# Lukeasargen/Show-Attend-and-Tell-Pytorch-Lightning

Hardware: AMD Instinct MI355X
Metric: captions/sec (train step) at B=128, 256px, seq_len=22 (higher is better)
Workload: dtype bf16; 1 GPU; C2: resnet50 encoder_size=7 encoder_dim=512 vocab=6400 T=22, 128 images/GPU x R=5 captions, trainable encoder, Adam, full lengths, decoder_tf=always; global_batch_images=128, parallelism=dp1, grad_bucket_dtype=fp32

## Files before the change

include/sat_hip.h:

```cpp
#ifndef SAT_HIP_H
#define SAT_HIP_H
#include <stddef.h>
#include <stdint.h>

#ifdef __cplusplus
extern "C" {
#endif

#define SAT_HIP_ABI_VERSION 23

int sat_abi_version(void);
int sat_debug_trace_launches(int32_t on);
int sat_debug_option(const char* name, int32_t value);
const char* sat_last_error(void);

typedef struct sat_profile_entry {
    char name[96];
    int64_t launches;
    double total_ms;
    double flops;
    double bytes;
} sat_profile_entry;
int sat_profile_start(void);
int sat_profile_start_only(const char* name);
int sat_profile_pause(int32_t paused);
int sat_profile_stop(sat_profile_entry* out, int32_t max_entries, int32_t* n_out);

typedef struct sat_gemm_desc {
    const float* A; int64_t lda; const int32_t* a_rows;
    const float* B; int64_t ldb;
    float* C; int64_t ldc;       const int32_t* c_rows;
    int32_t M, N, K;
    int32_t amode, bmode;
    int32_t accumulate;
    int32_t epi;
    const float* bias; const float* e0; int64_t lde0; int32_t c0, c1;
    float* slab; int64_t slab_elems;
} sat_gemm_desc;
int sat_gemm_f32(const sat_gemm_desc* d, void* stream);
typedef struct sat_gemm_types { int32_t a_bf16, b_bf16, c_bf16, bf16_mfma; } sat_gemm_types;
int sat_gemm_ex(const sat_gemm_desc* d, const sat_gemm_types* t, void* stream);

typedef struct sat_decoder_dims {
    int32_t B;
    int32_t R;
    int32_t T;
    int32_t L;
    int32_t D;
    int32_t A;
    int32_t m;
    int32_t n;
    int32_t V;
    int32_t P;
    int32_t deep_output;
    int32_t padding_idx;
    int32_t precision;
    int32_t layers;
    float embed_max_norm;
    float dropout;
    float embedding_dropout;
    uint64_t dropout_seed;
} sat_decoder_dims;

#define SAT_MAX_LSTM_LAYERS 4
typedef struct sat_decoder_params {
    float* embedding;
    float* init_f_w; float* init_f_b;
    float* init_i_w; float* init_i_b;
    float* w_ih; float* w_hh;
    float* b_ih; float* b_hh;
    float* att_enc;
    float* att_dec;
    float* att_f;
    float* beta_w; float* beta_b;
    float* out_hidden;
    float* out_context;
    float* out_w; float* out_b;
    float* up_w_ih[SAT_MAX_LSTM_LAYERS - 1]; float* up_w_hh[SAT_MAX_LSTM_LAYERS - 1];
    float* up_b_ih[SAT_MAX_LSTM_LAYERS - 1]; float* up_b_hh[SAT_MAX_LSTM_LAYERS - 1];
} sat_decoder_params;

typedef struct sat_decoder_batch {
    const float* ann;
    const int32_t* caps;
    const int32_t* lengths;
    const int32_t* prow;
    const int32_t* src_row;
    const int32_t* step_offsets_host;
    const int32_t* teacher_host;
} sat_decoder_batch;

size_t sat_decoder_workspace_bytes(const sat_decoder_dims* d);

int sat_decoder_train_fwd(const sat_decoder_dims* d, const sat_decoder_params* w, const sat_decoder_batch* b,
                          float* logits_packed, float* alphas, void* workspace, size_t workspace_bytes, void* stream);

int sat_decoder_train_bwd(const sat_decoder_dims* d, const sat_decoder_params* w, const sat_decoder_batch* b,
                          const float* dlogits_packed, const float* alphas , const float* dalphas,
                          const sat_decoder_params* g, float* dann, void* workspace, size_t workspace_bytes, void* stream);

int sat_decoder_train_bwd_fork(const sat_decoder_dims* d, const sat_decoder_params* w, const sat_decoder_batch* b,
                               const float* dlogits_packed, const float* alphas, const float* dalphas, const sat_decoder_params* g,
                               float* dann, void* workspace, size_t workspace_bytes, void* side_stream, void* event, void* stream);

int sat_ce_label_smooth_fwd(const float* logits, const int32_t* targets, int32_t P, int32_t V, float smoothing,
                            float* lse_rows, float* loss_rows, int32_t* correct_rows, float* out, void* stream);
int sat_ce_label_smooth_bwd(const float* logits, const int32_t* targets, const float* lse_rows, int32_t P, int32_t V,
                            float smoothing, const float* gscale, float* dlogits, void* stream);
int sat_doubly_stochastic_fwd(const float* alphas, int32_t N, int32_t T1, int32_t L, float gamma,
                              float* asum, float* part, float* out, void* stream);
int sat_doubly_stochastic_bwd(const float* asum, const float* gscale, int32_t N, int32_t T1, int32_t L, float gamma,
                              float* dalphas, void* stream);

int sat_policy_nll_fwd(const float* logits, const int32_t* targets, const float* row_weight, int32_t P, int32_t V, float inv_temperature,
                       const int32_t* masked_ids, int32_t n_first_rows, float scale, float* lse_rows, float* logq_rows, float* out, void* stream);
int sat_policy_nll_bwd(const float* logits, const int32_t* targets, const float* row_weight, const float* lse_rows, int32_t P, int32_t V,
                       float inv_temperature, const int32_t* masked_ids, int32_t n_first_rows, float scale, const float* gscale, float* dlogits,
                       void* stream);
#define SAT_SCST_BASELINE_GREEDY 0
#define SAT_SCST_BASELINE_MEAN 1
#define SAT_SCST_MAX_SAMPLES 256
int sat_scst_prepare(const int32_t* cap_tokens, const int32_t* cap_len, const double* scores, const double* scores_greedy , int32_t B,
                     int32_t K, int32_t S, double w_cider, double w_rouge, int32_t baseline_mode, const int32_t* special_ids_host, float* reward,
                     float* baseline , float* advantage, int32_t* caps, int32_t* lengths, float* step_weight, int32_t* count,
                     void* stream);

int sat_distill_fwd(const float* logits, const float* const* teachers, const float* weights, int32_t members, int32_t combine, const int32_t* targets,
                    int32_t P, int32_t V, float inv_tau, float alpha, float smoothing, float* lse_rows, float* teacher_lse_rows, float* cnorm_rows,
                    float* loss_rows, int32_t* correct_rows, float* out, float* dlogits , void* stream);
int sat_distill_bwd(const float* logits, const float* const* teachers, const float* weights, int32_t members, int32_t combine, const int32_t* targets,
                    int32_t P, int32_t V, float inv_tau, float alpha, float smoothing, const float* lse_rows, const float* teacher_lse_rows,
                    const float* cnorm_rows, const float* gscale, int32_t dlogits_from_fwd, float* dlogits, void* stream);

#define SAT_TEMPERATURE_MAX 8
size_t sat_temperature_workspace_bytes(int32_t P, int32_t V);
int sat_temperature_nll(const float* logits, const int32_t* targets, int32_t P, int32_t V, const float* temperatures,
                        int32_t n_temperatures, float* loss_out, float* grad_out, void* workspace, void* stream);
int sat_temperature_fit(const float* logits, const int32_t* targets, int32_t P, int32_t V, float init, float lr, float momentum,
                        int32_t nesterov, int32_t iters, float* t_trace, float* loss_trace, void* workspace, void* stream);

size_t sat_decoder_infer_workspace_bytes(const sat_decoder_dims* d, int32_t max_beams);
int sat_decoder_infer_begin(const sat_decoder_dims* d, const sat_decoder_params* w, const float* ann , int32_t beams,
                            int32_t max_beams, float* h , float* c, void* workspace, size_t workspace_bytes, void* stream);
int sat_decoder_infer_step(const sat_decoder_dims* d, const sat_decoder_params* w, const float* ann, const int32_t* tokens, int32_t beams,
                           int32_t max_beams, float* h, float* c, float* logits , float* alpha ,
// ... 489 lines not shown
```

show-attend-and-tell-pytorch-lightning_amd/_lib.py:

```python
import ctypes as C
import weakref
import os

import torch

_HERE = os.path.dirname(os.path.abspath(__file__))
LIB_PATH = os.path.join(_HERE, "libsat_hip.so")
_lib = None

f32p = C.POINTER(C.c_float)
i32p = C.POINTER(C.c_int32)


class GemmDesc(C.Structure):
    _fields_ = [("A", C.c_void_p), ("lda", C.c_int64), ("a_rows", C.c_void_p),
                ("B", C.c_void_p), ("ldb", C.c_int64),
                ("C", C.c_void_p), ("ldc", C.c_int64), ("c_rows", C.c_void_p),
                ("M", C.c_int32), ("N", C.c_int32), ("K", C.c_int32),
                ("amode", C.c_int32), ("bmode", C.c_int32), ("accumulate", C.c_int32), ("epi", C.c_int32),
                ("bias", C.c_void_p), ("e0", C.c_void_p), ("lde0", C.c_int64), ("c0", C.c_int32), ("c1", C.c_int32),
                ("slab", C.c_void_p), ("slab_elems", C.c_int64)]


class DecoderDims(C.Structure):
# ... 92 lines not shown


class BeamSearchOut(C.Structure):
    _fields_ = [(k, C.c_void_p) for k in SEARCH_OUTPUTS]


class ImageDesc(C.Structure):
    _fields_ = [("offset", C.c_int64)] + [(k, C.c_int32) for k in ("height", "width", "crop_top", "crop_left", "crop_h", "crop_w", "resized_h",
                                                                  "resized_w", "out_top", "out_left", "flip", "reserved")]


class ImageJitter(C.Structure):
    _fields_ = [("order", C.c_int32 * 4), ("brightness", C.c_float), ("contrast", C.c_float), ("saturation", C.c_float), ("hue_shift", C.c_int32)]


class ImageWarp(C.Structure):
    _fields_ = [("kind", C.c_int32), ("reserved", C.c_int32), ("coeffs", C.c_double * 8)]


class JpegDesc(C.Structure):
    _fields_ = [(k, C.c_int64) for k in ("data_offset", "data_bytes", "segments_offset", "out_offset", "block_offset")] + \
               [(k, C.c_int32) for k in ("height", "width", "components", "h_samp", "v_samp", "restart_interval", "n_segments", "segment_base")] + \
               [(k, C.c_int32 * 3) for k in ("quant", "dc_table", "ac_table")] + [("reserved", C.c_int32)]


class JpegDecodeOpts(C.Structure):
    _fields_ = [("subseq_bytes", C.c_int32), ("reserved", C.c_int32), ("parallel_min_bytes", C.c_int64), ("info", C.c_void_p)]


class JpegScan(C.Structure):
    _fields_ = [(k, C.c_int64) for k in ("data_offset", "data_bytes", "segments_offset")] + \
               [("picture", C.c_int32), ("level", C.c_int32), ("n_components", C.c_int32), ("component", C.c_int32 * 3)] + \
               [(k, C.c_int32) for k in ("ss", "se", "ah", "al")] + [("dc_table", C.c_int32 * 3), ("ac_table", C.c_int32)] + \
               [(k, C.c_int32) for k in ("restart_interval", "n_segments", "segment_base", "reserved")]


class JpegQTable(C.Structure):
    _fields_ = [("q", C.c_uint16 * 64)]


class JpegHTable(C.Structure):
    _fields_ = [("lookup", C.c_uint16 * 512), ("maxcode", C.c_int32 * 18), ("valoffset", C.c_int32 * 18), ("huffval", C.c_uint8 * 256)]


class DecoderBatch(C.Structure):
    _fields_ = [("ann", C.c_void_p), ("caps", C.c_void_p), ("lengths", C.c_void_p), ("prow", C.c_void_p), ("src_row", C.c_void_p),
                ("step_offsets_host", C.c_void_p), ("teacher_host", C.c_void_p)]


SYMBOLS = {
    "sat_abi_version": (C.c_int, []),
    "sat_debug_trace_launches": (C.c_int, [C.c_int32]),
    "sat_debug_option": (C.c_int, [C.c_char_p, C.c_int32]),
    "sat_last_error": (C.c_char_p, []),
    "sat_gemm_f32": (C.c_int, [C.POINTER(GemmDesc), C.c_void_p]),
    "sat_decoder_workspace_bytes": (C.c_size_t, [C.POINTER(DecoderDims)]),
    "sat_decoder_train_fwd": (C.c_int, [C.POINTER(DecoderDims), C.POINTER(DecoderParams), C.POINTER(DecoderBatch),
                                        C.c_void_p, C.c_void_p, C.c_void_p, C.c_size_t, C.c_void_p]),
    "sat_decoder_train_bwd": (C.c_int, [C.POINTER(DecoderDims), C.POINTER(DecoderParams), C.POINTER(DecoderBatch),
                                        C.c_void_p, C.c_void_p, C.c_void_p, C.POINTER(DecoderParams), C.c_void_p,
                                        C.c_void_p, C.c_size_t, C.c_void_p]),
    "sat_decoder_train_bwd_fork": (C.c_int, [C.POINTER(DecoderDims), C.POINTER(DecoderParams), C.POINTER(DecoderBatch),
                                             C.c_void_p, C.c_void_p, C.c_void_p, C.POINTER(DecoderParams), C.c_void_p,
                                             C.c_void_p, C.c_size_t, C.c_void_p, C.c_void_p, C.c_void_p]),
    "sat_ce_label_smooth_fwd": (C.c_int, [C.c_void_p, C.c_void_p, C.c_int32, C.c_int32, C.c_float, C.c_void_p, C.c_void_p,
                                          C.c_void_p, C.c_void_p, C.c_void_p]),
    "sat_ce_label_smooth_bwd": (C.c_int, [C.c_void_p, C.c_void_p, C.c_void_p, C.c_int32, C.c_int32, C.c_float, C.c_void_p,
                                          C.c_void_p, C.c_void_p]),
    "sat_doubly_stochastic_fwd": (C.c_int, [C.c_void_p, C.c_int32, C.c_int32, C.c_int32, C.c_float, C.c_void_p, C.c_void_p,
                                            C.c_void_p, C.c_void_p]),
    "sat_doubly_stochastic_bwd": (C.c_int, [C.c_void_p, C.c_void_p, C.c_int32, C.c_int32, C.c_int32, C.c_float, C.c_void_p, C.c_void_p]),
    "sat_attention_precompute": (C.c_int, [C.c_void_p, C.c_void_p, C.c_void_p, C.c_int32, C.c_int32, C.c_int32, C.c_int32, C.c_void_p]),
    "sat_attention_step_fwd": (C.c_int, [C.c_void_p, C.c_void_p, C.c_void_p, C.c_int32, C.c_void_p, C.c_void_p, C.c_int32,
                                         C.c_void_p, C.c_int32, C.c_void_p, C.c_void_p, C.c_int32, C.c_int32, C.c_int32,
                                         C.c_int32, C.c_int32, C.c_void_p]),
}


class GemmTypes(C.Structure):
    _fields_ = [(k, C.c_int32) for k in ("a_bf16", "b_bf16", "c_bf16", "bf16_mfma")]


class ConvGeom(C.Structure):
    _fields_ = [(k, C.c_int32) for k in ("N", "H", "W", "C", "K", "R", "S", "stride", "pad", "stride_w")]


class BlockDesc(C.Structure):
    _fields_ = ([(k, C.c_int32) for k in ("kind", "stride", "cin", "mid", "cout", "has_ds", "N", "H", "W", "fwd_res_bn", "dgrad_join", "bn_bwd_epilogue")] +
                [(k, C.c_void_p) for k in ("w1", "w2", "w3", "wd")] +
                [("gamma", C.c_void_p * 4), ("beta", C.c_void_p * 4), ("running_mean", C.c_void_p * 4), ("running_var", C.c_void_p * 4),
                 ("eps", C.c_float * 4), ("momentum", C.c_float * 4)] +
                [(k, C.c_void_p) for k in ("dw1", "dw2", "dw3", "dwd")] + [("dgamma", C.c_void_p * 4), ("dbeta", C.c_void_p * 4)])


_vp, _i32, _i64, _f = C.c_void_p, C.c_int32, C.c_int64, C.c_float
SYMBOLS.update({
    "sat_encoder_blocks_arena_bytes": (C.c_size_t, [C.POINTER(BlockDesc), _i32]),
    "sat_encoder_blocks_fwd": (C.c_int, [C.POINTER(BlockDesc), _i32, _vp, _vp, C.c_size_t, _vp, C.POINTER(C.c_void_p), _vp]),
    "sat_encoder_blocks_bwd": (C.c_int, [C.POINTER(BlockDesc), _i32, _i32, _i32, _vp, _vp, C.c_size_t, _vp, _vp, _i32, _vp, _vp, _i64, _vp, _i64, _vp, _vp,
                                         C.POINTER(C.c_void_p), C.POINTER(C.c_void_p), C.POINTER(C.c_int32), _vp]),
    "sat_conv2d_fwd": (C.c_int, [_vp, _vp, _vp, _vp, C.POINTER(ConvGeom), _vp]),
    "sat_conv2d_dgrad": (C.c_int, [_vp, _vp, _vp, C.POINTER(ConvGeom), _i32, _vp]),
    "sat_conv2d_wgrad": (C.c_int, [_vp, _vp, _vp, C.POINTER(ConvGeom), _vp, _i64, _vp]),
    "sat_conv2d_wgrad_slab_bytes": (C.c_size_t, [C.POINTER(ConvGeom)]),
    "sat_conv2d_fwd_bf16": (C.c_int, [_vp, _vp, _vp, _vp, C.POINTER(ConvGeom), _vp]),
    "sat_conv2d_dgrad_bf16": (C.c_int, [_vp, _vp, _vp, C.POINTER(ConvGeom), _i32, _vp]),
    "sat_conv2d_wgrad_bf16": (C.c_int, [_vp, _vp, _vp, C.POINTER(ConvGeom), _vp, _i64, _vp]),
    "sat_gemm_ex": (C.c_int, [C.POINTER(GemmDesc), C.POINTER(GemmTypes), _vp]),
    "sat_image_normalize_nhwc4": (C.c_int, [_vp, _vp, _i32, _i32, _i32, C.POINTER(C.c_float), C.POINTER(C.c_float), _vp]),
# ... 286 lines not shown
```

show-attend-and-tell-pytorch-lightning_amd/csrc/api.hip:

```cpp
#include <stdarg.h>

#include "../../include/sat_hip.h"
#include "decoder.h"
#include "gemm.h"
#include "gemm_bf16_common.h"
#include "temperature.h"
#include "caption_score.h"

namespace sat {
static thread_local char g_err[512] = {0};
int& dev_switch(int which) {
    static int v[SW_COUNT] = {0 , getenv("SAT_NO_WGRAD3X3") ? !atoi(getenv("SAT_NO_WGRAD3X3")) : 1,
                              getenv("SAT_REDUCE_Z16") ? atoi(getenv("SAT_REDUCE_Z16")) : 1, getenv("SAT_WIDE_TILES") ? atoi(getenv("SAT_WIDE_TILES")) : 0,
                              getenv("SAT_BN_ONEPASS") ? atoi(getenv("SAT_BN_ONEPASS")) : 1,
                              getenv("SAT_BN_VPT") ? atoi(getenv("SAT_BN_VPT")) : 2,
                              getenv("SAT_ACC_PREFETCH") ? atoi(getenv("SAT_ACC_PREFETCH")) : 0};
    return v[which];
}
int& trace_launches() { static int on = getenv("SAT_TRACE_LAUNCH") ? 1 : 0; return on; }
char* last_error_buf() { return g_err; }
int fail(int code, const char* fmt, ...) {
    va_list ap; va_start(ap, fmt); vsnprintf(g_err, sizeof g_err, fmt, ap); va_end(ap);
    return code;
}
}

using namespace sat;

extern "C" {

int sat_abi_version(void) { return SAT_HIP_ABI_VERSION; }
int sat_debug_trace_launches(int32_t on) { sat::trace_launches() = on ? 1 : 0; return SAT_OK; }
int sat_debug_option(const char* name, int32_t value) {
    if (!name) return fail(SAT_EINVAL, "debug_option: null name");
    if (!strcmp(name, "wgrad3x3")) { dev_switch(SW_WGRAD3X3) = value; return SAT_OK; }
    if (!strcmp(name, "reduce_z16")) { dev_switch(SW_REDUCE_Z16) = value; return SAT_OK; }
    if (!strcmp(name, "acc_prefetch")) { dev_switch(SW_ACC_PREFETCH) = value; return SAT_OK; }
    if (!strcmp(name, "bn_vpt")) { dev_switch(SW_BN_VPT) = value; return SAT_OK; }
    if (!strcmp(name, "bn_onepass")) { dev_switch(SW_BN_ONEPASS) = value; return SAT_OK; }
    if (!strcmp(name, "wide_tiles")) { dev_switch(SW_WIDE_TILES) = value; return SAT_OK; }
    if (!strcmp(name, "glds_tile")) { glds_force_tile() = value; return SAT_OK; }
    if (!strcmp(name, "glds_stages8")) { glds_stages8() = value; return SAT_OK; }
    if (!strcmp(name, "glds_tall_k")) { glds_tall_k() = value; return SAT_OK; }
    if (!strcmp(name, "glds_tall_conv")) { glds_tall_conv() = value; return SAT_OK; }
    if (!strcmp(name, "tile_override")) { gemm_tile_override() = value; return SAT_OK; }
    return fail(SAT_EINVAL, "debug_option: unknown option %s", name);
}
const char* sat_last_error(void) { return last_error_buf(); }

static int gemm_from_desc(const sat_gemm_desc* d, const sat_gemm_types* t, void* stream);
int sat_gemm_f32(const sat_gemm_desc* d, void* stream) { return gemm_from_desc(d, nullptr, stream); }
int sat_gemm_ex(const sat_gemm_desc* d, const sat_gemm_types* t, void* stream) {
    if (!t) return fail(SAT_EINVAL, "sat_gemm_ex: null type descriptor");
    return gemm_from_desc(d, t, stream);
}
static int gemm_from_desc(const sat_gemm_desc* d, const sat_gemm_types* t, void* stream) {
    if (!d) return fail(SAT_EINVAL, "sat_gemm_f32: null descriptor");
    if (d->amode != A_ROW && d->amode != A_KMAJOR) return fail(SAT_EINVAL, "sat_gemm_f32: amode %d (dense modes only)", d->amode);
    if (d->bmode != B_ROW && d->bmode != B_KMAJOR) return fail(SAT_EINVAL, "sat_gemm_f32: bmode %d (dense modes only)", d->bmode);
    GemmArgs g;
    g.A = d->A; g.lda = d->lda; g.a_rows = d->a_rows; g.B = d->B; g.ldb = d->ldb; g.C = d->C; g.ldc = d->ldc; g.c_rows = d->c_rows;
    g.M = d->M; g.N = d->N; g.K = d->K; g.amode = d->amode; g.bmode = d->bmode; g.accumulate = d->accumulate; g.epi = d->epi;
    g.bias = d->bias; g.e0 = d->e0; g.lde0 = d->lde0; g.c0 = d->c0; g.c1 = d->c1; g.slab = d->slab; g.slab_elems = d->slab_elems;
    if (t) { g.a_bf16 = t->a_bf16; g.b_bf16 = t->b_bf16; g.c_bf16 = t->c_bf16; g.bf16_mfma = t->bf16_mfma; }
    return launch_gemm(g, (hipStream_t)stream);
}

size_t sat_decoder_workspace_bytes(const sat_decoder_dims* d) {
    if (check_dims(d) != SAT_OK) return 0;
    return decoder_workspace_bytes(*d);
}

static int check_params(const sat_decoder_dims* d, const sat_decoder_params* w, const char* what) {
    if (!w) return fail(SAT_EINVAL, "%s: null parameter struct", what);
    if (!w->embedding || !w->init_f_w || !w->init_f_b || !w->init_i_w || !w->init_i_b || !w->w_ih || !w->w_hh || !w->b_ih || !w->b_hh ||
        !w->att_enc || !w->att_dec || !w->att_f || !w->beta_w || !w->beta_b || !w->out_hidden || !w->out_w)
        return fail(SAT_EINVAL, "%s: null tensor in parameter struct", what);
    if (d->deep_output && !w->out_context) return fail(SAT_EINVAL, "%s: deep output needs output.context.weight", what);
    for (int l = 1; l < d->layers; ++l)
        if (!w->up_w_ih[l - 1] || !w->up_w_hh[l - 1] || !w->up_b_ih[l - 1] || !w->up_b_hh[l - 1])
            return fail(SAT_EINVAL, "%s: null tensor for LSTM layer %d", what, l);
    return SAT_OK;
}
static int check_batch(const sat_decoder_batch* b) {
    if (!b || !b->ann || !b->caps || !b->lengths || !b->prow || !b->src_row || !b->step_offsets_host || !b->teacher_host)
        return fail(SAT_EINVAL, "decoder: null field in batch struct");
    return SAT_OK;
}

int sat_decoder_train_fwd(const sat_decoder_dims* d, const sat_decoder_params* w, const sat_decoder_batch* b, float* logits_packed,
                          float* alphas, void* workspace, size_t workspace_bytes, void* stream) {
    SAT_TRY(check_dims(d)); SAT_TRY(check_params(d, w, "decoder_train_fwd")); SAT_TRY(check_batch(b));
    if (!alphas || !workspace || (d->P > 0 && !logits_packed)) return fail(SAT_EINVAL, "decoder_train_fwd: null output/workspace");
    return decoder_fwd(*d, *w, *b, logits_packed, alphas, (char*)workspace, workspace_bytes, (hipStream_t)stream);
}

int sat_decoder_train_bwd(const sat_decoder_dims* d, const sat_decoder_params* w, const sat_decoder_batch* b, const float* dlogits_packed,
                          const float* alphas, const float* dalphas, const sat_decoder_params* g, float* dann, void* workspace,
                          size_t workspace_bytes, void* stream) {
    SAT_TRY(check_dims(d)); SAT_TRY(check_params(d, w, "decoder_train_bwd")); SAT_TRY(check_params(d, g, "decoder_train_bwd(grads)")); SAT_TRY(check_batch(b));
    if (!alphas || !dann || !workspace || (d->P > 0 && !dlogits_packed)) return fail(SAT_EINVAL, "decoder_train_bwd: null input/output/workspace");
    return decoder_bwd(*d, *w, *b, dlogits_packed, alphas, dalphas, *g, dann, (char*)workspace, workspace_bytes, (hipStream_t)stream);
}

int sat_decoder_train_bwd_fork(const sat_decoder_dims* d, const sat_decoder_params* w, const sat_decoder_batch* b, const float* dlogits_packed,
                               const float* alphas, const float* dalphas, const sat_decoder_params* g, float* dann, void* workspace,
                               size_t workspace_bytes, void* side_stream, void* event, void* stream) {
    SAT_TRY(check_dims(d)); SAT_TRY(check_params(d, w, "decoder_train_bwd_fork")); SAT_TRY(check_params(d, g, "decoder_train_bwd_fork(grads)")); SAT_TRY(check_batch(b));
    if (!alphas || !dann || !workspace || (d->P > 0 && !dlogits_packed)) return fail(SAT_EINVAL, "decoder_train_bwd_fork: null input/output/workspace");
    if ((side_stream != nullptr) != (event != nullptr)) return fail(SAT_EINVAL, "decoder_train_bwd_fork: side stream and event go together (got %s only)", side_stream ? "a stream" : "an event");
    if (side_stream && side_stream == stream) return fail(SAT_EINVAL, "decoder_train_bwd_fork: the side stream is the caller's stream");
    if (workspace_bytes < decoder_workspace_bytes(*d))
        return fail(SAT_EINVAL, "decoder_train_bwd_fork: workspace %zu < %zu bytes", workspace_bytes, decoder_workspace_bytes(*d));
    return decoder_bwd(*d, *w, *b, dlogits_packed, alphas, dalphas, *g, dann, (char*)workspace, workspace_bytes, (hipStream_t)stream, (hipStream_t)side_stream,
                       (hipEvent_t)event);
}

int sat_ce_label_smooth_fwd(const float* logits, const int32_t* targets, int32_t P, int32_t V, float smoothing, float* lse_rows,
                            float* loss_rows, int32_t* correct_rows, float* out, void* stream) {
    if (!logits || !targets || !lse_rows || !loss_rows || !correct_rows || !out) return fail(SAT_EINVAL, "ce_label_smooth_fwd: null pointer");
    return ce_fwd(logits, targets, P, V, smoothing, lse_rows, loss_rows, correct_rows, out, (hipStream_t)stream);
}
int sat_ce_label_smooth_bwd(const float* logits, const int32_t* targets, const float* lse_rows, int32_t P, int32_t V, float smoothing,
// ... 496 lines not shown
```

show-attend-and-tell-pytorch-lightning_amd/csrc/decoder.h:

```cpp
#pragma once
#include "../../include/sat_hip.h"
#include "common.h"

namespace sat {
struct Ws;
int check_dims(const sat_decoder_dims* d);
size_t decoder_workspace_bytes(const sat_decoder_dims& d);
int decoder_fwd(const sat_decoder_dims& d, const sat_decoder_params& p, const sat_decoder_batch& b, float* logits, float* alphas,
                char* ws, size_t ws_bytes, hipStream_t st);
int decoder_bwd(const sat_decoder_dims& d, const sat_decoder_params& p, const sat_decoder_batch& b, const float* dlogits,
                const float* alphas, const float* dalphas, const sat_decoder_params& g, float* dann, char* ws, size_t ws_bytes, hipStream_t st,
                hipStream_t side = nullptr, hipEvent_t fork_event = nullptr);
enum { ATT_OP_FWD = 0, ATT_OP_BWD = 1, ATT_OP_CONTEXT_BWD = 2 };
enum { ATT_FORM_SPLIT = 0, ATT_FORM_SINGLE = 1 };
enum : unsigned { ATT_HAS_SCRATCH = 1, ATT_ANN_ALIGNED = 2, ATT_ROWS_ALIGNED = 4, ATT_HAS_BF16 = 8 };
struct AttPlan {
    int form = 0, rn = 0, passes = 0;
    int vw = 0, dchunk = 0;
    int nq = 0, lq = 0;
    size_t lds0 = 0, lds1 = 0;
};
int attention_plan(int op, int R, int L, int D, int A, int hc_ld, int T1, unsigned flags, AttPlan& plan, const char* who);
int launch_attention_fwd(hipStream_t st, const float* ann, const float* U, const float* hc, int hc_ld, const float* wf,
                         const int* lengths, int step, float* alphas, int T1, float* Z, float* XZ, int B, int R, int L, int D, int A, float* sc, void* xzb,
                         const void* annb);
size_t decoder_infer_workspace_bytes(const sat_decoder_dims& d, int Kmax);
int decoder_infer_begin(const sat_decoder_dims& d, const sat_decoder_params& p, const float* ann, int K, int Kmax, float* h, float* c,
                        char* ws, size_t ws_bytes, hipStream_t st);
int decoder_infer_step(const sat_decoder_dims& d, const sat_decoder_params& p, const float* ann, const int* tokens, int K, int Kmax,
                       float* h, float* c, float* logits, float* alpha, const float* h_noise, char* ws, size_t ws_bytes, hipStream_t st);
size_t decoder_beam_workspace_bytes(const sat_decoder_dims& d, int K, int topg, int hist_stride, int groups);
int beam_groups_check(const sat_beam_groups* g, const char* what);
bool beam_history_on(const sat_beam_history* h);
int beam_history_check(const sat_beam_history* h, int max_gen_length, const char* what);
int beam_search_workspace_bytes(const sat_beam_search_desc& s, size_t& total);
int beam_search(const sat_beam_search_desc& s, const sat_beam_search_out& o, char* ws, size_t ws_bytes, hipStream_t st);
int beam_required_check(const sat_beam_required* r, int K, int max_gen_length, const char* what);
int beam_ensemble_check_weights(const float* weight, int members, int combine, const char* what);
int beam_ensemble_check(const sat_beam_ensemble* e, const char* what);
size_t decoder_beam_ensemble_workspace_bytes(const sat_beam_ensemble& e, int K, int hist_stride);
int beam_ensemble_scores(const float* const* logits, const float* weight, int members, int combine, int rows, int V, float temperature, float* combined,
                         hipStream_t st);
int launch_attention_bwd(hipStream_t st, const float* ann, const float* U, const float* hc, int hc_ld, const float* wf, const int* lengths, int step,
                         const float* alphas, const float* dalphas, int T1, const float* Z, const float* dZ, const float* dXZ, float* DZ, float* dhc,
                         int dhc_ld, float* dU, float* dwf_part, float* da, int B, int R, int L, int D, int A, void* dhcb, const void* annb);
int attention_context_bwd(const float* alphas, const float* DZ, const int* lengths, float* dann, int accumulate, int B, int R, int T1, int L, int D, hipStream_t st);
int lstm_cell_fwd(const float* x, int in, const float* h_prev, const float* c_prev, const float* w_ih, const float* w_hh, const float* b_ih, const float* b_hh,
                  float* gates, float* h_new, float* c_new, float* bias_scratch, int N, int n, hipStream_t st);
int lstm_cell_bwd(const float* x, int in, const float* h_prev, const float* c_prev, const float* c_new, const float* gates, const float* dh_new, const float* dc_new,
                  const float* w_ih, const float* w_hh, float* dx, float* dh_prev, float* dc_prev, float* dw_ih, float* dw_hh, float* db_ih, float* db_hh,
                  float* dgates, float* scratch, int N, int n, hipStream_t st);
int deep_output_fwd(const float* prev_embed, const float* hidden, const float* context, const float* w_hidden, const float* w_context, const float* w_out,
                    const float* b_out, float dropout, unsigned long long seed, float* u, float* udrop, float* logits, int N, int m, int n, int D, int V, hipStream_t st);
int deep_output_bwd(const float* dlogits, const float* hidden, const float* context, const float* u, const float* udrop, const float* w_hidden, const float* w_context,
                    const float* w_out, float dropout, unsigned long long seed, float* d_prev_embed, float* d_hidden, float* d_context, float* dw_hidden,
                    float* dw_context, float* dw_out, float* db_out, float* scratch, int N, int m, int n, int D, int V, hipStream_t st);
int init_lstm_fwd(const float* ann, const float* w_f, const float* b_f, const float* w_i, const float* b_i, float dropout, unsigned long long seed, float* mean,
                  float* f, float* init, int N, int L, int D, int m, int n2, hipStream_t st);
int init_lstm_bwd(const float* dinit, const float* mean, const float* f, const float* w_f, const float* w_i, float dropout, unsigned long long seed, float* dw_f,
                  float* db_f, float* dw_i, float* db_i, float* dann, float* df, float* dmean, float* scratch, int N, int L, int D, int m, int n2, hipStream_t st);
int embedding_fwd(float* table, const int* tokens, float* out, int rows, int V, int m, float max_norm, int* flags, hipStream_t st);
int embedding_bwd(const float* dY, const int* tokens, float* dtable, int rows, int V, int m, int padding_idx, int* scratch, hipStream_t st);
int sigmoid_bwd(const float* dy, const float* y, float* dpre, long n, hipStream_t st);
int beam_scores(const float* logits, int K, int V, float temperature, const int* masked, int n_masked, const float* parent, float* scores, hipStream_t st);
int beam_history_scores(const float* logits, int rows, int V, float temperature, const int* masked, int n_masked, const float* parent, const int* hist,
                        const int* hist_len, int hist_stride, const sat_beam_history& rules, int step, int end_id, float* scores, hipStream_t st);
int beam_group_select(const float* scores, const int* klive, int B, int K, int G, int V, int first_step, float lambda, float* work, float* values, int* indices,
                      hipStream_t st);
int beam_required_select(const float* scores, const int* klive, int B, int K, int V, const int* hist, int hist_stride, int hist_len, int first_step,
                         const sat_beam_required& req, int end_id, float* work, float* values, int* indices, hipStream_t st);
int topk(const float* x, float* work, long n, int k, float* values, int* indices, hipStream_t st);
int nucleus_keys(const float* scores, int rows, int V, float topp, float step, unsigned long long seed, unsigned long long stream, const float* gumbel,
                 float* keys, int* nucleus_size, hipStream_t st);
int colsum_public(const float* x, long ld, long rows, int cols, float* out, float* scratch, hipStream_t st);
int ce_fwd(const float* logits, const int* targets, int P, int V, float smoothing, float* lse_rows, float* loss_rows, int* correct_rows, float* out, hipStream_t st);
int ce_bwd(const float* logits, const int* targets, const float* lse_rows, int P, int V, float smoothing, const float* gscale, float* dlogits, hipStream_t st);
int ds_fwd(const float* alphas, int N, int T1, int L, float gamma, float* asum, float* part, float* out, hipStream_t st);
int ds_bwd(const float* asum, const float* gscale, int N, int T1, int L, float gamma, float* dalphas, hipStream_t st);
}
```

show-attend-and-tell-pytorch-lightning_amd/csrc/decoder.hip:

```cpp
#include "../../include/sat_hip.h"
#include <stdlib.h>
#include <map>
#include <mutex>
#include <utility>
#include "decoder_step.h"
#include "profile.h"
#include "decoder_kernels.h"

namespace sat {

struct Ws {
    size_t total = 0;
    float *U, *mean, *f, *init_img, *H_all, *C_all, *HC, *Z, *XZ, *Y, *GY, *Uact, *Wcat, *bcat;
    float *Udrop, *mean_rows, *f_rows, *init_rows, *df_rows;
    float *GU, *DGU, *bup;
    __bf16 *Wb_out, *Ub;
    __bf16 *annb;
    __bf16 *Hb, *XZb, *Wcat_b, *Wz_b, *DHCb;
    int* Tok; int* flags;
    int *emb_count, *emb_offset, *emb_cursor, *emb_list;
    float *SC, *DA;
    float *dA, *dHout, *dZout, *DZ, *DHC, *dXZ, *dHc, *dCc, *dU, *dwf_part, *dY, *colpart, *dinit_img, *df, *dmean, *slab;
    float *dmean_rows;
    float *colpart2, *slab2;
    char *zero_begin, *zero_end;
    long slab_elems;
};

Ws layout(const sat_decoder_dims& d, char* base) {
    Ws w; size_t off = 0;
    const long N = (long)d.B * d.R, T1 = d.T - 1, HCW = d.A + d.D + 4L * d.n;
    auto take = [&](size_t elems, size_t esz = 4) { size_t o = off; off += (elems * esz + 255) & ~(size_t)255; return base ? base + o : (char*)nullptr; };
    w.U = (float*)take((size_t)d.B * d.L * d.A);
    w.mean = (float*)take((size_t)d.B * d.D);
    w.f = (float*)take((size_t)d.B * d.m);
    const int NL = d.layers;
    w.init_img = (float*)take((size_t)d.B * 2 * d.n * NL);
    w.H_all = (float*)take((size_t)NL * (T1 + 1) * N * d.n);
    w.C_all = (float*)take((size_t)NL * (T1 + 1) * N * d.n);
    w.GU = w.DGU = w.bup = nullptr;
    if (NL > 1) {
        w.GU = (float*)take((size_t)(NL - 1) * T1 * N * 4 * d.n); w.DGU = (float*)take((size_t)(NL - 1) * T1 * N * 4 * d.n);
        w.bup = (float*)take((size_t)(NL - 1) * 4 * d.n);
    }
    w.HC = (float*)take((size_t)T1 * N * HCW);
    w.Z = (float*)take((size_t)T1 * N * d.D);
    w.XZ = (float*)take((size_t)T1 * N * d.D);
    w.Y = (float*)take((size_t)T1 * N * d.m);
    w.GY = (float*)take((size_t)T1 * N * 4 * d.n);
    w.Uact = (float*)take((size_t)(d.P > 0 ? d.P : 1) * d.m);
    w.Wcat = (float*)take((size_t)HCW * d.n);
    w.bcat = (float*)take((size_t)HCW);
    w.Tok = (int*)take((size_t)T1 * N);
    w.Udrop = w.mean_rows = w.f_rows = w.init_rows = w.df_rows = w.dmean_rows = nullptr;
// ... 18 lines not shown
    w.emb_list = (int*)take((size_t)T1 * N);
    w.SC = (float*)take((size_t)N * d.L); w.DA = (float*)take((size_t)N * d.L);
    w.dA = (float*)take((size_t)(d.P > 0 ? d.P : 1) * d.m);
    w.DZ = (float*)take((size_t)T1 * N * d.D);
    w.DHC = (float*)take((size_t)T1 * N * HCW);
    w.dXZ = (float*)take((size_t)N * d.D);
    w.dHout = (float*)take((size_t)T1 * N * d.n); w.zero_begin = (char*)w.dHout;
    w.dZout = (float*)take((size_t)T1 * N * d.D);
    w.dHc = (float*)take((size_t)NL * N * d.n);
    w.dCc = (float*)take((size_t)NL * N * d.n);
    w.dU = (float*)take((size_t)d.B * d.L * d.A);
    w.dwf_part = (float*)take((size_t)d.B * d.A);
    w.zero_end = base ? base + off : (char*)nullptr;
    w.dY = (float*)take((size_t)T1 * N * d.m);
    long maxrows = d.P > T1 * N ? d.P : T1 * N; if (maxrows < d.B * (long)d.L) maxrows = d.B * (long)d.L;
    long maxcols = d.V > HCW ? d.V : HCW;
    w.colpart = (float*)take((size_t)cdiv(maxrows, 256) * maxcols);
    w.dinit_img = (float*)take((size_t)d.B * 2 * d.n * NL);
    w.df = (float*)take((size_t)d.B * d.m);
    w.dmean = (float*)take((size_t)d.B * d.D);
    w.slab_elems = 8L << 20;
    w.slab = (float*)take((size_t)w.slab_elems);
    w.colpart2 = (float*)take((size_t)cdiv(maxrows, 256) * maxcols);
    w.slab2 = (float*)take((size_t)w.slab_elems);
    w.total = off;
    return w;
}

int check_dims(const sat_decoder_dims* d) {
    SAT_REQUIRE(d, "decoder: null dims");
    SAT_REQUIRE(d->B > 0 && d->R > 0 && d->T >= 2 && d->L > 0 && d->D > 0 && d->A > 0 && d->m > 0 && d->n > 0 && d->V > 0,
                "decoder: non-positive dimension (B=%d R=%d T=%d L=%d D=%d A=%d m=%d n=%d V=%d)", d->B, d->R, d->T, d->L, d->D, d->A, d->m, d->n, d->V);
    SAT_REQUIRE(d->P >= 0 && (long)d->P <= (long)d->B * d->R * (d->T - 1), "decoder: packed token count %d out of range", d->P);
    SAT_REQUIRE(d->layers >= 1 && d->layers <= SAT_MAX_LSTM_LAYERS, "decoder: layers=%d outside 1..%d", d->layers, SAT_MAX_LSTM_LAYERS);
    SAT_REQUIRE(d->dropout >= 0.f && d->dropout < 1.f && d->embedding_dropout >= 0.f && d->embedding_dropout < 1.f, "decoder: dropout must lie in [0,1)");
    return SAT_OK;
}

thread_local int t_bf16_mfma = 0;

static int cast_bf16(hipStream_t st, const float* src, __bf16* dst, long n) {
    hipLaunchKernelGGL(cast_bf16_kernel, dim3(cdiv(n / 4, 256)), dim3(256), 0, st, src, dst, n / 4);
    return launch_ok("cast_bf16");
}
static int gemm_bb_nt(hipStream_t st, const __bf16* A, long lda, const __bf16* B, long ldb, float* C, long ldc, int M, int N, int K, int epi, const float* bias,
                      int acc = 0, int c0 = 0, int c1 = 0) {
    GemmArgs g;
    g.A = A; g.lda = lda; g.B = B; g.ldb = ldb; g.C = C; g.ldc = ldc; g.M = M; g.N = N; g.K = K;
    g.amode = A_ROW; g.bmode = B_ROW; g.epi = epi; g.bias = bias; g.a_bf16 = g.b_bf16 = 1; g.c_bf16 = 0; g.bf16_mfma = 1;
    g.accumulate = acc; g.c0 = c0; g.c1 = c1;
    return launch_gemm(g, st);
}

static int gemm_bb_nn(hipStream_t st, const __bf16* A, long lda, const __bf16* B, long ldb, float* C, long ldc, int M, int N, int K, int acc, float* slab, long slab_elems) {
    GemmArgs g;
    g.A = A; g.lda = lda; g.B = B; g.ldb = ldb; g.C = C; g.ldc = ldc; g.M = M; g.N = N; g.K = K;
    g.amode = A_ROW; g.bmode = B_KMAJOR; g.a_bf16 = g.b_bf16 = 1; g.c_bf16 = 0; g.bf16_mfma = 1; g.accumulate = acc; g.slab = slab; g.slab_elems = slab_elems;
    return launch_gemm(g, st);
}

static int colsum(hipStream_t st, const Ws& w, const float* x, long ld, int rows, int cols, float* out, int accumulate = 0, float scale = 1.f) {
    if (cols <= 0) return SAT_OK;
    if (rows <= 0) { if (!accumulate) SAT_TRY(dev_fill_bytes(st, out, 0, (size_t)cols * 4)); return SAT_OK; }
    int nparts = cdiv(rows, 256);
    if (cols % 4 == 0 && ld % 4 == 0 && (reinterpret_cast<uintptr_t>(x) & 15) == 0)
        hipLaunchKernelGGL(colsum_part4_kernel, dim3(cdiv(cols / 4, 128), nparts), dim3(128), 0, st, x, ld, rows, cols / 4, 256, w.colpart);
    else
        hipLaunchKernelGGL(colsum_part_kernel, dim3(cdiv(cols, 256), nparts), dim3(256), 0, st, x, ld, rows, cols, 256, w.colpart);
    SAT_TRY(launch_ok("colsum_part"));
    hipLaunchKernelGGL(colsum_finish_kernel, dim3(cdiv(cols, 256)), dim3(256), 0, st, w.colpart, nparts, cols, out, accumulate, scale);
    return launch_ok("colsum_finish");
}

int pack_step_weights(const sat_decoder_dims& d, const sat_decoder_params& p, float* Wcat, __bf16* Wcat_b, float* bcat, float* bup, hipStream_t st) {
    const int n = d.n, HCW = d.A + d.D + 4 * n;
    hipLaunchKernelGGL(pack_wcat_kernel, dim3(cdiv((long)HCW * n + HCW, 256)), dim3(256), 0, st, p.att_dec, p.beta_w, p.w_hh, p.beta_b, p.b_ih, p.b_hh, Wcat, Wcat_b,
                       bcat, d.A, d.D, n);
    SAT_TRY(launch_ok("pack Wcat"));
    for (int l = 1; l < d.layers; ++l) {
        hipLaunchKernelGGL(add_kernel, dim3(cdiv(4 * n, 256)), dim3(256), 0, st, bup + (long)(l - 1) * 4 * n, p.up_b_ih[l - 1], p.up_b_hh[l - 1], (long)4 * n);
        SAT_TRY(launch_ok("bias add (stacked layer)"));
    }
    return SAT_OK;
}
int image_begin(const sat_decoder_dims& d, const sat_decoder_params& p, const float* ann, int images, float* U, float* mean, float* f, float* init_img,
                hipStream_t st) {
    const int n2 = 2 * d.n * d.layers;
    SAT_TRY(gemm(st, A_ROW, B_ROW, ann, d.D, p.att_enc, d.D, U, d.A, images * d.L, d.A, d.D));
    hipLaunchKernelGGL(ann_mean_kernel, dim3(images), dim3(256), 0, st, ann, mean, d.L, d.D);
    SAT_TRY(launch_ok("ann_mean"));
    if (!f) return SAT_OK;
    SAT_TRY(gemm(st, A_ROW, B_ROW, mean, d.D, p.init_f_w, d.D, f, d.m, images, d.m, d.D, 0, EPI_BIAS, p.init_f_b));
    return gemm(st, A_ROW, B_ROW, f, d.m, p.init_i_w, d.m, init_img, n2, images, n2, d.m, 0, EPI_BIAS, p.init_i_b);
}
int lstm_cell_pointwise(float* gates, int g_ld, const float* c_prev, const float* h_prev, float* c_new, float* h_new, const int* live, int rows, int n,
                        hipStream_t st) {
    hipLaunchKernelGGL(lstm_cell_fwd_kernel, dim3(cdiv((long)rows * n, 256)), dim3(256), 0, st, gates, g_ld, (const float*)nullptr, c_prev, h_prev, c_new, h_new, live,
                       0, rows, n, (__bf16*)nullptr);
    return launch_ok("lstm_cell_fwd");
}

static int live_steps(const sat_decoder_dims& d, const sat_decoder_batch& b) {
    const int T1 = d.T - 1; int ts = 0;
    for (int t = 0; t < T1; ++t) if (b.step_offsets_host[t + 1] > b.step_offsets_host[t]) ts = t + 1;
    return ts;
}

static size_t att_fwd_lds(int L, int A, int vw) { return (size_t)(ATT_RMAX * L + ATT_RMAX * A + A + ATT_RMAX * ATT_THREADS * vw) * 4; }
static size_t att_bwd_lds(int L, int A, int D) { return (size_t)(2 * ATT_RMAX * L + ATT_RMAX * A + A + ATT_RMAX * D + ATTB_WAVES * ATT_RMAX * A + ATTB_WAVES * A) * 4; }

// ... 82 lines not shown

int launch_attention_fwd(hipStream_t st, const float* ann, const float* U, const float* hc, int hc_ld, const float* wf,
                                const int* lengths, int step, float* alphas, int T1, float* Z, float* XZ, int B, int R, int L, int D, int A, float* sc, void* xzb_v,
                                const void* annb_v) {
    __bf16* xzb = reinterpret_cast<__bf16*>(xzb_v);
    const __bf16* annb = reinterpret_cast<const __bf16*>(annb_v);
    static const int no_split = getenv("SAT_ATT_FUSED") ? atoi(getenv("SAT_ATT_FUSED")) : 0;
    const unsigned flags = (sc && !no_split ? ATT_HAS_SCRATCH : 0u) | (al16(ann) && (!annb || al8(annb)) ? ATT_ANN_ALIGNED : 0u) |
                           (al16(hc) && al16(Z) && al16(XZ) ? ATT_ROWS_ALIGNED : 0u) | (xzb || annb ? ATT_HAS_BF16 : 0u);
    AttPlan pl;
    SAT_TRY(attention_plan(ATT_OP_FWD, R, L, D, A, hc_ld, T1, flags, pl, "attention_fwd"));
    if (pl.form == ATT_FORM_SPLIT) {
        switch (pl.rn) {
            case 1: return annb ? attention_fwd_split<1, __bf16>(st, annb, U, hc, hc_ld, wf, lengths, step, alphas, T1, Z, XZ, B, R, L, D, A, sc, xzb, pl)
                                : attention_fwd_split<1, float>(st, ann, U, hc, hc_ld, wf, lengths, step, alphas, T1, Z, XZ, B, R, L, D, A, sc, xzb, pl);
            case 2: return annb ? attention_fwd_split<2, __bf16>(st, annb, U, hc, hc_ld, wf, lengths, step, alphas, T1, Z, XZ, B, R, L, D, A, sc, xzb, pl)
                                : attention_fwd_split<2, float>(st, ann, U, hc, hc_ld, wf, lengths, step, alphas, T1, Z, XZ, B, R, L, D, A, sc, xzb, pl);
            case 3: return annb ? attention_fwd_split<3, __bf16>(st, annb, U, hc, hc_ld, wf, lengths, step, alphas, T1, Z, XZ, B, R, L, D, A, sc, xzb, pl)
                                : attention_fwd_split<3, float>(st, ann, U, hc, hc_ld, wf, lengths, step, alphas, T1, Z, XZ, B, R, L, D, A, sc, xzb, pl);
            case 4: return annb ? attention_fwd_split<4, __bf16>(st, annb, U, hc, hc_ld, wf, lengths, step, alphas, T1, Z, XZ, B, R, L, D, A, sc, xzb, pl)
                                : attention_fwd_split<4, float>(st, ann, U, hc, hc_ld, wf, lengths, step, alphas, T1, Z, XZ, B, R, L, D, A, sc, xzb, pl);
            case 5: return annb ? attention_fwd_split<5, __bf16>(st, annb, U, hc, hc_ld, wf, lengths, step, alphas, T1, Z, XZ, B, R, L, D, A, sc, xzb, pl)
                                : attention_fwd_split<5, float>(st, ann, U, hc, hc_ld, wf, lengths, step, alphas, T1, Z, XZ, B, R, L, D, A, sc, xzb, pl);
            case 6: return annb ? attention_fwd_split<6, __bf16>(st, annb, U, hc, hc_ld, wf, lengths, step, alphas, T1, Z, XZ, B, R, L, D, A, sc, xzb, pl)
                                : attention_fwd_split<6, float>(st, ann, U, hc, hc_ld, wf, lengths, step, alphas, T1, Z, XZ, B, R, L, D, A, sc, xzb, pl);
            case 7: return annb ? attention_fwd_split<7, __bf16>(st, annb, U, hc, hc_ld, wf, lengths, step, alphas, T1, Z, XZ, B, R, L, D, A, sc, xzb, pl)
                                : attention_fwd_split<7, float>(st, ann, U, hc, hc_ld, wf, lengths, step, alphas, T1, Z, XZ, B, R, L, D, A, sc, xzb, pl);
            default: return annb ? attention_fwd_split<8, __bf16>(st, annb, U, hc, hc_ld, wf, lengths, step, alphas, T1, Z, XZ, B, R, L, D, A, sc, xzb, pl)
                                 : attention_fwd_split<8, float>(st, ann, U, hc, hc_ld, wf, lengths, step, alphas, T1, Z, XZ, B, R, L, D, A, sc, xzb, pl);
        }
    }
    const bool vec = pl.vw == 4;
    const int dchunk = pl.dchunk;
    const size_t lds = pl.lds0;
    dim3 grid(B, cdiv(D, dchunk));
    const int RN = pl.rn;
#define SAT_ATTF(VWV, RNV)                                                                                                                  \
    case RNV:                                                                                                                               \
        SAT_TRY(ensure_dynamic_lds(reinterpret_cast<const void*>(attention_fwd_kernel<VWV, RNV>), lds)); \
        hipLaunchKernelGGL((attention_fwd_kernel<VWV, RNV>), grid, dim3(ATTF_THREADS), lds, st, ann, U, hc, hc_ld, wf, lengths, step, alphas, T1, Z, XZ, R, L, D, A, dchunk); \
        break;
    if (vec) {
        switch (RN) { SAT_ATTF(4, 1) SAT_ATTF(4, 2) SAT_ATTF(4, 3) SAT_ATTF(4, 4) SAT_ATTF(4, 5) SAT_ATTF(4, 6) SAT_ATTF(4, 7) SAT_ATTF(4, 8) default: break; }
    } else {
        switch (RN) { SAT_ATTF(1, 1) SAT_ATTF(1, 2) SAT_ATTF(1, 3) SAT_ATTF(1, 4) SAT_ATTF(1, 5) SAT_ATTF(1, 6) SAT_ATTF(1, 7) SAT_ATTF(1, 8) default: break; }
    }
#undef SAT_ATTF
    return launch_ok("attention_fwd");
}

template <int RN, typename TA>
static int attention_bwd_split_t(hipStream_t st, const TA* ann, const float* U, const float* hc, int hc_ld, const float* wf, const int* lengths, int step,
                                 const float* alphas, const float* dalphas, int T1, const float* Zs, const float* dZ_out, const float* dXZ, float* DZ, float* dhc,
                                 int dhc_ld, float* dU, float* dwf_part, float* da, int B, int R, int L, int D, int A, __bf16* dhcb, const AttPlan& pl) {
    const size_t lds_a = pl.lds0, lds_t = pl.lds1;
    SAT_TRY(ensure_dynamic_lds(reinterpret_cast<const void*>(attention_bwd_dalpha_kernel<RN, TA>), lds_a));
    SAT_TRY(ensure_dynamic_lds(reinterpret_cast<const void*>(attention_bwd_tanh_kernel<RN>), lds_t));
    const double N = (double)B * R;
    {
        ProfScope prof("attention_bwd_dalpha", 2.0 * N * L * D, (double)sizeof(TA) * B * L * D + 4.0 * N * (5.0 * D + 2.0 * L), st);
        hipLaunchKernelGGL((attention_bwd_dalpha_kernel<RN, TA>), dim3(B, cdiv(L, 16)), dim3(1024), lds_a, st, ann, hc, hc_ld, lengths, step, dalphas, T1, Zs, dZ_out, dXZ, DZ, dhc,
                           dhc_ld, da, R, L, D, A, dhcb);
        SAT_TRY(launch_ok("attention_bwd_dalpha"));
    }
    ProfScope prof("attention_bwd_tanh", 4.0 * N * L * A, 4.0 * (3.0 * B * L * A + N * (2.0 * A + 2.0 * L)), st);
    hipLaunchKernelGGL(attention_bwd_tanh_kernel<RN>, dim3(B, cdiv(A, ATTB_KCH)), dim3(1024), lds_t, st, U, hc, hc_ld, wf, lengths, step, alphas, T1, da, dhc, dhc_ld, dU,
                       dwf_part, R, L, A, dhcb);
    return launch_ok("attention_bwd_tanh");
}
int launch_attention_bwd(hipStream_t st, const float* ann, const float* U, const float* hc, int hc_ld, const float* wf, const int* lengths, int step,
                         const float* alphas, const float* dalphas, int T1, const float* Zs, const float* dZ_out, const float* dXZ, float* DZ, float* dhc,
                         int dhc_ld, float* dU, float* dwf_part, float* da, int B, int R, int L, int D, int A, void* dhcb_v, const void* annb_v) {
    __bf16* dhcb = reinterpret_cast<__bf16*>(dhcb_v);
    const __bf16* annb = reinterpret_cast<const __bf16*>(annb_v);
    const unsigned flags = (da ? ATT_HAS_SCRATCH : 0u) | (al16(ann) && (!annb || al8(annb)) ? ATT_ANN_ALIGNED : 0u) | (dhcb || annb ? ATT_HAS_BF16 : 0u);
    AttPlan pl;
    SAT_TRY(attention_plan(ATT_OP_BWD, R, L, D, A, hc_ld, T1, flags, pl, "attention_bwd"));
    SAT_REQUIRE(dhc_ld >= A + D, "attention_bwd: dhc_ld %d < A+D", dhc_ld);
    if (pl.form == ATT_FORM_SPLIT) {
#define SAT_ATTB(RNV) case RNV: return annb ? attention_bwd_split_t<RNV, __bf16>(st, annb, U, hc, hc_ld, wf, lengths, step, alphas, dalphas, T1, Zs, dZ_out, dXZ, DZ, dhc, dhc_ld, dU, dwf_part, da, B, R, L, D, A, dhcb, pl) \
                                            : attention_bwd_split_t<RNV, float>(st, ann, U, hc, hc_ld, wf, lengths, step, alphas, dalphas, T1, Zs, dZ_out, dXZ, DZ, dhc, dhc_ld, dU, dwf_part, da, B, R, L, D, A, dhcb, pl);
        switch (pl.rn) { SAT_ATTB(1) SAT_ATTB(2) SAT_ATTB(3) SAT_ATTB(4) SAT_ATTB(5) SAT_ATTB(6) SAT_ATTB(7) default: SAT_ATTB(8) }
#undef SAT_ATTB
    }
    typedef void (*attb_fn)(const float*, const float*, const float*, int, const float*, const int*, int, const float*, const float*, int, const float*,
                            const float*, const float*, float*, float*, int, float*, float*, int, int, int, int);
    attb_fn attb = nullptr;
    switch (pl.rn) {
        case 1: attb = attention_bwd_kernel<1>; break; case 2: attb = attention_bwd_kernel<2>; break; case 3: attb = attention_bwd_kernel<3>; break;
        case 4: attb = attention_bwd_kernel<4>; break; case 5: attb = attention_bwd_kernel<5>; break; case 6: attb = attention_bwd_kernel<6>; break;
        case 7: attb = attention_bwd_kernel<7>; break; default: attb = attention_bwd_kernel<8>; break;
    }
    SAT_TRY(ensure_dynamic_lds(reinterpret_cast<const void*>(attb), pl.lds0));
    hipLaunchKernelGGL(attb, dim3(B), dim3(ATTB_THREADS), pl.lds0, st, ann, U, hc, hc_ld, wf, lengths, step, alphas, dalphas, T1, Zs, dZ_out, dXZ, DZ, dhc, dhc_ld,
                       dU, dwf_part, R, L, D, A);
    return launch_ok("attention_bwd");
}

static int flush_outputs(hipStream_t st, const sat_decoder_dims& d, const sat_decoder_params& p, const sat_decoder_batch& b,
                         const Ws& w, float* logits, int p0, int p1) {
    const int rows = p1 - p0;
    if (rows <= 0) return SAT_OK;
    const long N = (long)d.B * d.R;
    const float* H1 = w.H_all + ((long)(d.layers - 1) * d.T + 1) * N * d.n;
    float* u = w.Uact + (long)p0 * d.m;
    const int* rows_map = b.src_row + p0;
    if (d.deep_output) {
        SAT_TRY(gemm(st, A_ROW, B_ROW, H1, d.n, p.out_hidden, d.n, u, d.m, rows, d.m, d.n, 0, EPI_NONE, nullptr, rows_map));
        SAT_TRY(gemm(st, A_ROW, B_ROW, w.Z, d.D, p.out_context, d.D, u, d.m, rows, d.m, d.D, 1, EPI_ADD_TANH, nullptr, rows_map, nullptr, w.Y, d.m));
    } else {
        SAT_TRY(gemm(st, A_ROW, B_ROW, H1, d.n, p.out_hidden, d.n, u, d.m, rows, d.m, d.n, 0, EPI_NONE, nullptr, rows_map));
    }
    const float* uin = u;
    if (d.dropout > 0.f) {
        float* ud = w.Udrop + (long)p0 * d.m;
        hipLaunchKernelGGL(dropout_rows_kernel, dim3(cdiv((long)rows * d.m, 256)), dim3(256), 0, st, u, ud, (long)rows * d.m, d.m, d.dropout,
                           (unsigned long long)d.dropout_seed, 2u, (long)p0);
        SAT_TRY(launch_ok("output dropout"));
        uin = ud;
    }
    if (w.Wb_out) {
        if (p0 == 0 || (p.out_w == p.embedding && d.embed_max_norm > 0.f)) SAT_TRY(cast_bf16(st, p.out_w, w.Wb_out, (long)d.V * d.m));
        SAT_TRY(cast_bf16(st, uin, w.Ub + (long)p0 * d.m, (long)rows * d.m));
        return gemm_bb_nt(st, w.Ub + (long)p0 * d.m, d.m, w.Wb_out, d.m, logits + (long)p0 * d.V, d.V, rows, d.V, d.m, p.out_b ? EPI_BIAS : EPI_NONE, p.out_b);
    }
    return gemm(st, A_ROW, B_ROW, uin, d.m, p.out_w, d.m, logits + (long)p0 * d.V, d.V, rows, d.V, d.m, 0,
                p.out_b ? EPI_BIAS : EPI_NONE, p.out_b);
}

int decoder_fwd(const sat_decoder_dims& d, const sat_decoder_params& p, const sat_decoder_batch& b, float* logits, float* alphas,
                       char* ws, size_t ws_bytes, hipStream_t st) {
    Ws w = layout(d, ws);
    t_bf16_mfma = d.precision ? 1 : 0;
    SAT_REQUIRE(ws_bytes >= w.total, "decoder_fwd: workspace %zu < %zu bytes", ws_bytes, w.total);
// ... 126 lines not shown
    auto Hs = [&](int t, int l) { return w.H_all + l * LS + (long)t * N * n; };
    auto Cs = [&](int t, int l) { return w.C_all + l * LS + (long)t * N * n; };
    auto GUs = [&](int t, int l) { return w.GU + ((long)(l - 1) * T1 + t) * N * 4 * n; };
    auto DGUs = [&](int t, int l) { return w.DGU + ((long)(l - 1) * T1 + t) * N * 4 * n; };
    auto dHcs = [&](int l) { return w.dHc + (long)l * N * n; };
    auto dCcs = [&](int l) { return w.dCc + (long)l * N * n; };
    float* const slab = w.slab; const long se = w.slab_elems;

    SAT_TRY(dev_fill_bytes(st, w.zero_begin, 0, (size_t)(w.zero_end - w.zero_begin)));
    if (NL > 1 && KR < T1 * N) SAT_TRY(dev_fill_bytes(st, w.DGU, 0, (size_t)(NL - 1) * T1 * N * 4 * n * 4));

    float* const lslab = wl.slab;
    auto leaf_out_w = [&]() -> int {
        if (P > 0) {
            SAT_TRY(gemm(ls, A_KMAJOR, B_KMAJOR, dlogits, V, d.dropout > 0.f ? w.Udrop : w.Uact, m, g.out_w, m, V, m, P, 0, EPI_NONE, nullptr, nullptr, nullptr, nullptr, 0, 0, 0, lslab, se));
            if (g.out_b) SAT_TRY(colsum(ls, wl, dlogits, V, P, V, g.out_b));
        } else {
            SAT_TRY(dev_fill_bytes(ls, g.out_w, 0, (size_t)V * m * 4));
            if (g.out_b) SAT_TRY(dev_fill_bytes(ls, g.out_b, 0, (size_t)V * 4));
        }
        return SAT_OK;
    };
    auto leaf_out_hidden = [&]() -> int {
        const float* H1 = Hs(1, top);
        SAT_TRY(gemm(ls, A_KMAJOR, B_KMAJOR, w.dY, m, H1, n, g.out_hidden, n, m, n, KR, 0, EPI_NONE, nullptr, nullptr, nullptr, nullptr, 0, 0, 0, lslab, se));
        if (d.deep_output)
            SAT_TRY(gemm(ls, A_KMAJOR, B_KMAJOR, w.dY, m, w.Z, D, g.out_context, D, m, D, KR, 0, EPI_NONE, nullptr, nullptr, nullptr, nullptr, 0, 0, 0, lslab, se));
        else
            SAT_TRY(dev_fill_bytes(ls, w.dY, 0, (size_t)T1 * N * m * 4));
        return SAT_OK;
    };
    if (P > 0) {
        SAT_TRY(gemm(st, A_ROW, B_KMAJOR, dlogits, V, p.out_w, m, w.dA, m, P, m, V, 0, d.deep_output ? EPI_MUL_DTANH : EPI_NONE, nullptr,
                     nullptr, nullptr, w.Uact, m, 0, 0, slab, se));
        if (d.dropout > 0.f) {
            hipLaunchKernelGGL(dropout_rows_kernel, dim3(cdiv((long)P * m, 256)), dim3(256), 0, st, w.dA, w.dA, (long)P * m, m, d.dropout,
                               (unsigned long long)d.dropout_seed, 2u, 0L);
            SAT_TRY(launch_ok("output dropout bwd"));
        }
    }
    if (!fork) SAT_TRY(leaf_out_w());
    if (P > 0) {
        SAT_TRY(gemm(st, A_ROW, B_KMAJOR, w.dA, m, p.out_hidden, n, w.dHout, n, P, n, m, 0, EPI_NONE, nullptr, nullptr, b.src_row));
        if (d.deep_output)
            SAT_TRY(gemm(st, A_ROW, B_KMAJOR, w.dA, m, p.out_context, D, w.dZout, D, P, D, m, 0, EPI_NONE, nullptr, nullptr, b.src_row));
    }
    hipLaunchKernelGGL(scatter_rows_kernel, dim3(T1 * N), dim3(64), 0, st, w.dA, b.prow, w.dY, T1 * N, m);
    SAT_TRY(launch_ok("scatter dA"));
    if (!fork) SAT_TRY(leaf_out_hidden());

    static const int att_fused = getenv("SAT_ATT_FUSED") ? atoi(getenv("SAT_ATT_FUSED")) : 0;
    const bool use_b = w.Hb != nullptr && !att_fused;
    const __bf16* annb = (w.annb && !att_fused && ann_bf16_enabled() && al16(b.ann)) ? w.annb : nullptr;
    for (int t = ts - 1; t >= 0; --t) {
        const float* hc = w.HC + (long)t * N * HCW;
        float* dhc = w.DHC + (long)t * N * HCW;
        for (int l = top; l >= 1; --l) {
            float* dgu = DGUs(t, l);
            hipLaunchKernelGGL(lstm_cell_bwd_kernel, dim3(cdiv((long)N * n, 256)), dim3(256), 0, st, GUs(t, l), 4 * n, Cs(t, l), Cs(t + 1, l),
                               l == top ? w.dHout + (long)t * N * n : (const float*)nullptr, dHcs(l), dCcs(l), dgu, 4 * n, b.lengths, t, N, n);
            SAT_TRY(launch_ok("lstm_cell_bwd (stacked layer)"));
            SAT_TRY(gemm(st, A_ROW, B_KMAJOR, dgu, 4 * n, p.up_w_ih[l - 1], n, dHcs(l - 1), n, N, n, 4 * n, 1, EPI_NONE, nullptr, nullptr, nullptr, nullptr, 0, 0, 0, slab, se));
            SAT_TRY(gemm(st, A_ROW, B_KMAJOR, dgu, 4 * n, p.up_w_hh[l - 1], n, dHcs(l), n, N, n, 4 * n, 1, EPI_NONE, nullptr, nullptr, nullptr, nullptr, 0, 0, 0, slab, se));
        }
        hipLaunchKernelGGL(lstm_cell_bwd_kernel, dim3(cdiv((long)N * n, 256)), dim3(256), 0, st, hc + A + D, HCW, Cs(t, 0),
                           Cs(t + 1, 0), top == 0 ? w.dHout + (long)t * N * n : (const float*)nullptr, dHcs(0), dCcs(0), dhc + A + D, HCW, b.lengths, t, N, n,
                           use_b ? w.DHCb + A + D : (__bf16*)nullptr);
        SAT_TRY(launch_ok("lstm_cell_bwd"));
        if (use_b) SAT_TRY(gemm_bb_nn(st, w.DHCb + A + D, HCW, w.Wz_b, D, w.dXZ, D, N, D, 4 * n, 0, slab, se));
        else SAT_TRY(gemm(st, A_ROW, B_KMAJOR, dhc + A + D, HCW, p.w_ih + m, m + D, w.dXZ, D, N, D, 4 * n, 0, EPI_NONE, nullptr, nullptr, nullptr, nullptr, 0, 0, 0, slab, se));
        SAT_TRY(launch_attention_bwd(st, b.ann, w.U, hc, HCW, p.att_f, b.lengths, t, alphas, dalphas, T1, w.Z + (long)t * N * D, w.dZout + (long)t * N * D, w.dXZ,
                                     w.DZ + (long)t * N * D, dhc, HCW, w.dU, w.dwf_part, att_fused ? nullptr : w.DA, d.B, d.R, d.L, D, A,
                                     use_b ? w.DHCb : nullptr, annb));
        if (use_b) {
            SAT_TRY(gemm_bb_nn(st, w.DHCb, HCW, w.Wcat_b, n, w.dHc, n, N, n, HCW, 1, slab, se));
        } else if (NL == 1) {
            SAT_TRY(gemm(st, A_ROW, B_KMAJOR, dhc, HCW, w.Wcat, n, w.dHc, n, N, n, HCW, 1, EPI_NONE, nullptr, nullptr, nullptr, nullptr, 0, 0, 0, slab, se));
        } else {
            SAT_TRY(gemm(st, A_ROW, B_KMAJOR, dhc, HCW, w.Wcat, n, dHcs(top), n, N, n, A + D, 1, EPI_NONE, nullptr, nullptr, nullptr, nullptr, 0, 0, 0, slab, se));
            SAT_TRY(gemm(st, A_ROW, B_KMAJOR, dhc + A + D, HCW, w.Wcat + (long)(A + D) * n, n, dHcs(0), n, N, n, 4 * n, 1, EPI_NONE, nullptr, nullptr, nullptr, nullptr, 0, 0, 0, slab, se));
        }
    }

    auto wgrad = [&](const float* dy, long ldy, const float* x, long ldx, float* out, long ldo, int M, int Nn) {
        return gemm(ls, A_KMAJOR, B_KMAJOR, dy, ldy, x, ldx, out, ldo, M, Nn, KR, 0, EPI_NONE, nullptr, nullptr, nullptr, nullptr, 0, 0, 0, lslab, se);
    };
    const float* dG = w.DHC + A + D;
    auto leaf_loop_params = [&]() -> int {
        SAT_TRY(wgrad(w.DHC, HCW, Hs(0, top), n, g.att_dec, n, A, n));
        SAT_TRY(wgrad(w.DHC + A, HCW, Hs(0, top), n, g.beta_w, n, D, n));
        SAT_TRY(wgrad(dG, HCW, Hs(0, 0), n, g.w_hh, n, 4 * n, n));
        for (int l = 1; l < NL; ++l) {
            const float* dgu = DGUs(0, l);
            SAT_TRY(wgrad(dgu, 4 * n, Hs(1, l - 1), n, g.up_w_ih[l - 1], n, 4 * n, n));
            SAT_TRY(wgrad(dgu, 4 * n, Hs(0, l), n, g.up_w_hh[l - 1], n, 4 * n, n));
            SAT_TRY(colsum(ls, wl, dgu, 4 * n, KR, 4 * n, g.up_b_ih[l - 1]));
            SAT_TRY(dev_copy_bytes(ls, g.up_b_hh[l - 1], g.up_b_ih[l - 1], (size_t)4 * n * 4));
        }
        SAT_TRY(colsum(ls, wl, w.DHC + A, HCW, KR, D, g.beta_b));
        SAT_TRY(colsum(ls, wl, dG, HCW, KR, 4 * n, g.b_ih));
        SAT_TRY(dev_copy_bytes(ls, g.b_hh, g.b_ih, (size_t)4 * n * 4));
        SAT_TRY(wgrad(dG, HCW, w.Y, m, g.w_ih, m + D, 4 * n, m));
        SAT_TRY(wgrad(dG, HCW, w.XZ, D, g.w_ih + m, m + D, 4 * n, D));
        SAT_TRY(gemm(ls, A_ROW, B_KMAJOR, dG, HCW, p.w_ih, m + D, w.dY, m, KR, m, 4 * n, 1));
        if (d.embedding_dropout > 0.f && KR > 0) {
            hipLaunchKernelGGL(dropout_rows_kernel, dim3(cdiv((long)KR * m, 256)), dim3(256), 0, ls, w.dY, w.dY, (long)KR * m, m, d.embedding_dropout,
                               (unsigned long long)d.dropout_seed, 1u, 0L);
            SAT_TRY(launch_ok("embedding dropout bwd"));
        }
        if (KR > 0) {
            SAT_TRY(dev_fill_bytes(ls, w.emb_count, 0, (size_t)V * 4));
            hipLaunchKernelGGL(embedding_count_kernel, dim3(cdiv(KR, 256)), dim3(256), 0, ls, w.Tok, KR, V, d.padding_idx, w.emb_count);
            hipLaunchKernelGGL(embedding_scan_kernel, dim3(1), dim3(1024), 0, ls, w.emb_count, V, w.emb_offset, w.emb_cursor);
            hipLaunchKernelGGL(embedding_place_kernel, dim3(cdiv(KR, 256)), dim3(256), 0, ls, w.Tok, KR, V, d.padding_idx, w.emb_offset, w.emb_cursor, w.emb_list);
            hipLaunchKernelGGL(embedding_sum_kernel, dim3(V), dim3(256), 0, ls, w.dY, w.Tok, w.emb_offset, w.emb_list, g.embedding, KR, m, d.padding_idx);
            SAT_TRY(launch_ok("embedding gradient"));
        } else SAT_TRY(dev_fill_bytes(ls, g.embedding, 0, (size_t)V * m * 4));
        SAT_TRY(colsum(ls, wl, w.dwf_part, A, d.B, A, g.att_f));
        return gemm(ls, A_KMAJOR, B_KMAJOR, w.dU, A, b.ann, D, g.att_enc, D, A, D, d.B * d.L, 0, EPI_NONE, nullptr, nullptr, nullptr, nullptr, 0, 0, 0, lslab, se);
    };
    auto crit_dann = [&]() -> int {
        SAT_TRY(gemm(st, A_ROW, B_KMAJOR, w.dU, A, p.att_enc, D, dann, D, d.B * d.L, D, A));
        return attention_context_bwd(alphas, w.DZ, b.lengths, dann, 1, d.B, d.R, T1, d.L, D, st);
    };
    const bool rows = d.dropout > 0.f;
    const int n2 = 2 * n * NL, IR = rows ? N : d.B;
    const float* dinit = rows ? w.init_rows : w.dinit_img;
    float* dfp = rows ? w.df_rows : w.df;
    auto crit_dinit = [&]() -> int {
        if (rows) {
// ... 4 lines not shown
        return launch_ok("init_expand_bwd");
    };
    auto leaf_init_i = [&]() -> int {
        SAT_TRY(gemm(ls, A_KMAJOR, B_KMAJOR, dinit, n2, rows ? w.f_rows : w.f, m, g.init_i_w, m, n2, m, IR));
        return colsum(ls, wl, dinit, n2, IR, n2, g.init_i_b);
    };
    auto crit_df = [&]() -> int { return gemm(st, A_ROW, B_KMAJOR, dinit, n2, p.init_i_w, m, dfp, m, IR, m, n2); };
    auto leaf_init_f = [&]() -> int {
        SAT_TRY(gemm(ls, A_KMAJOR, B_KMAJOR, dfp, m, rows ? w.mean_rows : w.mean, D, g.init_f_w, D, m, D, IR));
        return colsum(ls, wl, dfp, m, IR, m, g.init_f_b);
    };
    auto crit_dmean = [&]() -> int {
        if (rows) {
            SAT_TRY(gemm(st, A_ROW, B_KMAJOR, w.df_rows, m, p.init_f_w, D, w.dmean_rows, D, N, D, m));
            hipLaunchKernelGGL(init_mean_rows_bwd_kernel, dim3(cdiv((long)d.B * D, 256)), dim3(256), 0, st, w.dmean_rows, w.dmean, d.B, d.R, D, d.dropout,
                               (unsigned long long)d.dropout_seed);
            SAT_TRY(launch_ok("init_mean_rows_bwd"));
        } else {
            SAT_TRY(gemm(st, A_ROW, B_KMAJOR, w.df, m, p.init_f_w, D, w.dmean, D, d.B, D, m));
        }
        const long tot = (long)d.B * d.L * D;
        hipLaunchKernelGGL(dann_add_mean_kernel, dim3(cdiv(tot, 256)), dim3(256), 0, st, dann, w.dmean, d.L, D, tot);
        return launch_ok("dann_add_mean");
    };
    if (!fork) {
        SAT_TRY(leaf_loop_params());
        SAT_TRY(crit_dann());
        SAT_TRY(crit_dinit());
        SAT_TRY(leaf_init_i());
        SAT_TRY(crit_df());
        SAT_TRY(leaf_init_f());
        return crit_dmean();
    }
    SAT_TRY(crit_dann());
    SAT_TRY(crit_dinit());
    SAT_TRY(crit_df());
    SAT_CHECK_HIP(hipEventRecord(fork_event, st));
    SAT_TRY(crit_dmean());
    SAT_CHECK_HIP(hipStreamWaitEvent(side, fork_event, 0));
    SAT_TRY(leaf_out_w());
    SAT_TRY(leaf_out_hidden());
    SAT_TRY(leaf_loop_params());
    SAT_TRY(leaf_init_i());
    return leaf_init_f();
}


int colsum_public(const float* x, long ld, long rows, int cols, float* out, float* scratch, hipStream_t st) {
    Ws w; w.colpart = scratch;
    return colsum(st, w, x, ld, (int)rows, cols, out);
}

size_t decoder_workspace_bytes(const sat_decoder_dims& d) { return layout(d, nullptr).total; }


static int fill_f(hipStream_t st, float* p, long n, float v) {
    if (n <= 0) return SAT_OK;
    hipLaunchKernelGGL(fill_kernel, dim3(cdiv(n, 256)), dim3(256), 0, st, p, n, v);
    return launch_ok("fill");
}

int attention_context_bwd(const float* alphas, const float* DZ, const int* lengths, float* dann, int accumulate, int B, int R, int T1, int L, int D, hipStream_t st) {
    AttPlan pl;
    SAT_TRY(attention_plan(ATT_OP_CONTEXT_BWD, R, L, D, 0, 0, T1, 0u, pl, "attention_context_bwd"));
    const size_t lds = pl.lds0;
    if (pl.nq == 13) {
        SAT_TRY(ensure_dynamic_lds(reinterpret_cast<const void*>(dann_from_context_kernel<13>), lds));
        hipLaunchKernelGGL(dann_from_context_kernel<13>, dim3(B, cdiv(D, 256)), dim3(256), lds, st, alphas, DZ, lengths, dann, accumulate, R, B * R, T1, L, D);
    } else {
        SAT_TRY(ensure_dynamic_lds(reinterpret_cast<const void*>(dann_from_context_kernel<16>), lds));
        hipLaunchKernelGGL(dann_from_context_kernel<16>, dim3(B, cdiv(D, 256)), dim3(256), lds, st, alphas, DZ, lengths, dann, accumulate, R, B * R, T1, L, D);
    }
    return launch_ok("dann_from_context");
}

int lstm_cell_fwd(const float* x, int in, const float* h_prev, const float* c_prev, const float* w_ih, const float* w_hh, const float* b_ih, const float* b_hh,
                  float* gates, float* h_new, float* c_new, float* bias_scratch, int N, int n, hipStream_t st) {
    t_bf16_mfma = 0;
    hipLaunchKernelGGL(add_kernel, dim3(cdiv(4 * n, 256)), dim3(256), 0, st, bias_scratch, b_ih, b_hh, (long)4 * n);
    SAT_TRY(launch_ok("bias add"));
    SAT_TRY(gemm(st, A_ROW, B_ROW, x, in, w_ih, in, gates, 4 * n, N, 4 * n, in, 0, EPI_BIAS, bias_scratch));
    SAT_TRY(gemm(st, A_ROW, B_ROW, h_prev, n, w_hh, n, gates, 4 * n, N, 4 * n, n, 1));
    return lstm_cell_pointwise(gates, 4 * n, c_prev, h_prev, c_new, h_new, nullptr, N, n, st);
}

int lstm_cell_bwd(const float* x, int in, const float* h_prev, const float* c_prev, const float* c_new, const float* gates, const float* dh_new, const float* dc_new,
                  const float* w_ih, const float* w_hh, float* dx, float* dh_prev, float* dc_prev, float* dw_ih, float* dw_hh, float* db_ih, float* db_hh,
                  float* dgates, float* scratch, int N, int n, hipStream_t st) {
    t_bf16_mfma = 0;
    if (dc_new) SAT_TRY(dev_copy_bytes(st, dc_prev, dc_new, (size_t)N * n * 4));
    else SAT_TRY(fill_f(st, dc_prev, (long)N * n, 0.f));
    SAT_TRY(fill_f(st, dh_prev, (long)N * n, 0.f));
    hipLaunchKernelGGL(lstm_cell_bwd_kernel, dim3(cdiv((long)N * n, 256)), dim3(256), 0, st, gates, 4 * n, c_prev, c_new, dh_new, dh_prev, dc_prev, dgates, 4 * n,
                       (const int*)nullptr, 0, N, n, (__bf16*)nullptr);
    SAT_TRY(launch_ok("lstm_cell_bwd"));
    SAT_TRY(gemm(st, A_ROW, B_KMAJOR, dgates, 4 * n, w_ih, in, dx, in, N, in, 4 * n));
    SAT_TRY(gemm(st, A_ROW, B_KMAJOR, dgates, 4 * n, w_hh, n, dh_prev, n, N, n, 4 * n));
    SAT_TRY(gemm(st, A_KMAJOR, B_KMAJOR, dgates, 4 * n, x, in, dw_ih, in, 4 * n, in, N));
    SAT_TRY(gemm(st, A_KMAJOR, B_KMAJOR, dgates, 4 * n, h_prev, n, dw_hh, n, 4 * n, n, N));
    Ws w; w.colpart = scratch;
    SAT_TRY(colsum(st, w, dgates, 4 * n, N, 4 * n, db_ih));
    SAT_TRY(dev_copy_bytes(st, db_hh, db_ih, (size_t)4 * n * 4));
    return SAT_OK;
}

int deep_output_fwd(const float* prev_embed, const float* hidden, const float* context, const float* w_hidden, const float* w_context, const float* w_out,
                    const float* b_out, float dropout, unsigned long long seed, float* u, float* udrop, float* logits, int N, int m, int n, int D, int V, hipStream_t st) {
    t_bf16_mfma = 0;
    if (context) {
        SAT_TRY(gemm(st, A_ROW, B_ROW, hidden, n, w_hidden, n, u, m, N, m, n));
        SAT_TRY(gemm(st, A_ROW, B_ROW, context, D, w_context, D, u, m, N, m, D, 1, EPI_ADD_TANH, nullptr, nullptr, nullptr, prev_embed, m));
    } else {
        SAT_TRY(gemm(st, A_ROW, B_ROW, hidden, n, w_hidden, n, u, m, N, m, n));
    }
    const float* uin = u;
    if (dropout > 0.f) {
        hipLaunchKernelGGL(dropout_rows_kernel, dim3(cdiv((long)N * m, 256)), dim3(256), 0, st, u, udrop, (long)N * m, m, dropout, seed, 2u, 0L);
        SAT_TRY(launch_ok("output dropout"));
        uin = udrop;
    }
    return gemm(st, A_ROW, B_ROW, uin, m, w_out, m, logits, V, N, V, m, 0, b_out ? EPI_BIAS : EPI_NONE, b_out);
}

int deep_output_bwd(const float* dlogits, const float* hidden, const float* context, const float* u, const float* udrop, const float* w_hidden, const float* w_context,
                    const float* w_out, float dropout, unsigned long long seed, float* d_prev_embed, float* d_hidden, float* d_context, float* dw_hidden,
// ... 87 lines not shown
```

show-attend-and-tell-pytorch-lightning_amd/csrc/decoder_kernels.h:

```cpp
#pragma once
#include "common.h"
#include "row_reduce.h"

namespace sat {

constexpr int ATT_RMAX = 8;
constexpr int ATT_THREADS = 256;

__global__ void fill_kernel(float* p, long n, float v) {
    long i = (long)blockIdx.x * blockDim.x + threadIdx.x;
    if (i < n) p[i] = v;
}

__global__ void cast_bf16_kernel(const float* __restrict__ src, __bf16* __restrict__ dst, long n4) {
    long e = (long)blockIdx.x * blockDim.x + threadIdx.x;
    if (e >= n4) return;
    const float4 v = reinterpret_cast<const float4*>(src)[e];
    typedef __bf16 b4 __attribute__((ext_vector_type(4)));
    b4 o; o[0] = (__bf16)v.x; o[1] = (__bf16)v.y; o[2] = (__bf16)v.z; o[3] = (__bf16)v.w;
    reinterpret_cast<b4*>(dst)[e] = o;
}

__global__ void cast_block_bf16_kernel(const float* __restrict__ src, long ld, __bf16* __restrict__ dst, int rows, int cols) {
    long e = (long)blockIdx.x * blockDim.x + threadIdx.x;
// ... 374 lines not shown
            }
        }
#pragma unroll
        for (int r = 0; r < RN; ++r) s_part[(g * RN + r) * 16 + v] = acc[r];
        __syncthreads();
        for (int e = tid; e < rn * 16; e += 256) {
            const int r = e >> 4, vv = e & 15, dd = d0 + 4 * vv;
            if (dd >= D) continue;
            float4 z = make_float4(0.f, 0.f, 0.f, 0.f);
            for (int gg = 0; gg < 16; ++gg) { const float4 t = s_part[(gg * RN + r) * 16 + vv]; z.x += t.x; z.y += t.y; z.z += t.z; z.w += t.w; }
            const long orow = i0 + r;
            float4 be = make_float4(0.f, 0.f, 0.f, 0.f);
            if ((lmask >> r) & 1u) be = *reinterpret_cast<const float4*>(hc + orow * hc_ld + A + dd);
            *reinterpret_cast<float4*>(Z + orow * D + dd) = z;
            *reinterpret_cast<float4*>(XZ + orow * D + dd) = make_float4(be.x * z.x, be.y * z.y, be.z * z.z, be.w * z.w);
            if (xzb) {
                typedef __bf16 b4 __attribute__((ext_vector_type(4)));
                b4 o; o[0] = (__bf16)(be.x * z.x); o[1] = (__bf16)(be.y * z.y); o[2] = (__bf16)(be.z * z.z); o[3] = (__bf16)(be.w * z.w);
                *reinterpret_cast<b4*>(xzb + orow * D + dd) = o;
            }
        }
    }
}

__global__ void lstm_cell_fwd_kernel(float* __restrict__ gates, int g_ld, const float* __restrict__ gy,
                                     const float* __restrict__ c_prev, const float* __restrict__ h_prev,
                                     float* __restrict__ c_new, float* __restrict__ h_new,
                                     const int* __restrict__ lengths, int step, int N, int n, __bf16* __restrict__ hb_new = nullptr) {
    long idx = (long)blockIdx.x * blockDim.x + threadIdx.x;
    if (idx >= (long)N * n) return;
    int i = (int)(idx / n), j = (int)(idx - (long)i * n);
    if (lengths && lengths[i] <= step) {
        const float hp = h_prev[idx];
        c_new[idx] = c_prev[idx]; h_new[idx] = hp;
        if (hb_new) hb_new[idx] = (__bf16)hp;
        float* g = gates + (long)i * g_ld;
        g[j] = 0.f; g[n + j] = 0.f; g[2 * n + j] = 0.f; g[3 * n + j] = 0.f;
        return;
    }
    float* g = gates + (long)i * g_ld;
    const float* y = gy ? gy + (long)i * 4 * n : nullptr;
    float gi = fast_sigmoid(g[j] + (y ? y[j] : 0.f));
    float gf = fast_sigmoid(g[n + j] + (y ? y[n + j] : 0.f));
    float gg = fast_tanh(g[2 * n + j] + (y ? y[2 * n + j] : 0.f));
    float go = fast_sigmoid(g[3 * n + j] + (y ? y[3 * n + j] : 0.f));
    float c = gf * c_prev[idx] + gi * gg;
    c_new[idx] = c;
    const float hn = go * fast_tanh(c);
    h_new[idx] = hn;
    if (hb_new) hb_new[idx] = (__bf16)hn;
    g[j] = gi; g[n + j] = gf; g[2 * n + j] = gg; g[3 * n + j] = go;
}

__global__ void lstm_cell_bwd_kernel(const float* __restrict__ gates, int g_ld, const float* __restrict__ c_prev,
                                     const float* __restrict__ c_new, const float* __restrict__ dh_out,
                                     float* __restrict__ dh_carry, float* __restrict__ dc_carry,
                                     float* __restrict__ dgates, int dg_ld,
                                     const int* __restrict__ lengths, int step, int N, int n, __bf16* __restrict__ dgb = nullptr) {
    long idx = (long)blockIdx.x * blockDim.x + threadIdx.x;
    if (idx >= (long)N * n) return;
    int i = (int)(idx / n), j = (int)(idx - (long)i * n);
    float* dg = dgates + (long)i * dg_ld;
    __bf16* db = dgb ? dgb + (long)i * dg_ld : nullptr;
    if (lengths && lengths[i] <= step) {
        dg[j] = 0.f; dg[n + j] = 0.f; dg[2 * n + j] = 0.f; dg[3 * n + j] = 0.f;
        if (db) { db[j] = (__bf16)0.f; db[n + j] = (__bf16)0.f; db[2 * n + j] = (__bf16)0.f; db[3 * n + j] = (__bf16)0.f; }
        return;
    }
    const float* g = gates + (long)i * g_ld;
    float gi = g[j], gf = g[n + j], gg = g[2 * n + j], go = g[3 * n + j];
    float dh = dh_carry[idx] + (dh_out ? dh_out[idx] : 0.f);
    float tc = fast_tanh(c_new[idx]);
    float dc = dc_carry[idx] + dh * go * (1.f - tc * tc);
    const float d0 = dc * gg * gi * (1.f - gi), d1 = dc * c_prev[idx] * gf * (1.f - gf), d2 = dc * gi * (1.f - gg * gg), d3 = dh * tc * go * (1.f - go);
    dg[j] = d0; dg[n + j] = d1; dg[2 * n + j] = d2; dg[3 * n + j] = d3;
    if (db) { db[j] = (__bf16)d0; db[n + j] = (__bf16)d1; db[2 * n + j] = (__bf16)d2; db[3 * n + j] = (__bf16)d3; }
    dc_carry[idx] = dc * gf;
    dh_carry[idx] = 0.f;
}

constexpr int ATTB_WAVES = 16;
constexpr int ATTB_THREADS = ATTB_WAVES * 64;
template <int RN>
__global__ __launch_bounds__(ATTB_THREADS) void attention_bwd_kernel(
    const float* __restrict__ ann, const float* __restrict__ U, const float* __restrict__ hc, int hc_ld,
    const float* __restrict__ wf, const int* __restrict__ lengths, int step,
    const float* __restrict__ alphas, const float* __restrict__ dalphas_ext, int T1,
    const float* __restrict__ Zs, const float* __restrict__ dZ_out, const float* __restrict__ dXZ,
    float* __restrict__ DZ, float* __restrict__ dhc, int dhc_ld, float* __restrict__ dU, float* __restrict__ dwf_part,
    int R, int L, int D, int A) {
    extern __shared__ __attribute__((aligned(16))) float sm[];
    float* s_al = sm;
    float* s_da = s_al + ATT_RMAX * L;
    float* s_q = s_da + ATT_RMAX * L;
    float* s_w = s_q + ATT_RMAX * A;
    float* s_dz = s_w + A;
    float* s_dq = s_dz + ATT_RMAX * D;
    float* s_dw = s_dq + ATTB_WAVES * ATT_RMAX * A;
    const int b = blockIdx.x, tid = threadIdx.x, lane = tid & 63, wave = tid >> 6;
    const float scale = 1.0f / sqrtf((float)L);
    for (int k = tid; k < A; k += ATTB_THREADS) s_w[k] = wf[k];
    for (int e = tid; e < ATTB_WAVES * A; e += ATTB_THREADS) s_dw[e] = 0.f;

    for (int r0 = 0; r0 < R; r0 += RN) {
        const int rn = min(RN, R - r0);
        const int i0 = b * R + r0;
        unsigned lmask = 0;
        for (int r = 0; r < rn; ++r) if (lengths[i0 + r] > step) lmask |= 1u << r;
        const bool any = lmask != 0;
        __syncthreads();
        for (int e = tid; e < RN * D; e += ATTB_THREADS) {
            int r = e / D, d = e - r * D; long row = i0 + r;
            float dz = 0.f, dbp = 0.f;
            if (((lmask >> r) & 1u)) {
// ... 27 lines not shown
                if (lane == 0) s_da[r * L + l] = ((lmask >> r) & 1u) ? s + (dalphas_ext ? dalphas_ext[((long)(i0 + r) * T1 + step) * L + l] : 0.f) : 0.f;
            }
        }
        __syncthreads();
        for (int r = wave; r < rn; r += ATTB_WAVES) {
            if (!((lmask >> r) & 1u)) continue;
            float dot = 0.f;
            for (int l = lane; l < L; l += 64) dot += s_al[r * L + l] * s_da[r * L + l];
            dot = wave_sum(dot);
            for (int l = lane; l < L; l += 64) s_da[r * L + l] = s_al[r * L + l] * (s_da[r * L + l] - dot) * scale;
        }
        __syncthreads();
        for (int k0 = 0; k0 < A; k0 += 64) {
            const int k = k0 + lane;
            float dq[RN]; float dw = 0.f;
#pragma unroll
            for (int r = 0; r < RN; ++r) dq[r] = 0.f;
            if (k < A) {
                const float w = s_w[k];
                for (int l = wave; l < L; l += ATTB_WAVES) {
                    const long uo = ((long)b * L + l) * A + k;
                    const float uv = U[uo];
                    float du = 0.f;
#pragma unroll
                    for (int r = 0; r < RN; ++r) {
                        float th = fast_tanh(uv + s_q[r * A + k]);
                        float ds = s_da[r * L + l];
                        float dp = ds * w * (1.f - th * th);
                        dq[r] += dp; du += dp; dw = fmaf(ds, th, dw);
                    }
                    dU[uo] += du;
                }
#pragma unroll
                for (int r = 0; r < RN; ++r) s_dq[(wave * ATT_RMAX + r) * A + k] = dq[r];
                s_dw[wave * A + k] += dw;
            }
        }
        __syncthreads();
        for (int e = tid; e < rn * A; e += ATTB_THREADS) {
            int r = e / A, k = e - r * A;
            float s = 0.f;
            if (((lmask >> r) & 1u)) for (int w = 0; w < ATTB_WAVES; ++w) s += s_dq[(w * ATT_RMAX + r) * A + k];
            dhc[(long)(i0 + r) * dhc_ld + k] = s;
        }
    }
    __syncthreads();
    for (int k = tid; k < A; k += ATTB_THREADS) { float sw = 0.f; for (int w = 0; w < ATTB_WAVES; ++w) sw += s_dw[w * A + k]; dwf_part[(long)b * A + k] += sw; }
}

template <int RN, typename TA>
__global__ __launch_bounds__(1024) void attention_bwd_dalpha_kernel(const TA* __restrict__ ann, const float* __restrict__ hc, int hc_ld,
        const int* __restrict__ lengths, int step, const float* __restrict__ dalphas_ext, int T1, const float* __restrict__ Zs,
        const float* __restrict__ dZ_out, const float* __restrict__ dXZ, float* __restrict__ DZ, float* __restrict__ dhc, int dhc_ld,
        float* __restrict__ da, int R, int L, int D, int A, __bf16* __restrict__ dhcb) {
    extern __shared__ __attribute__((aligned(16))) float s_dz[];
    const int b = blockIdx.x, tid = threadIdx.x, lane = tid & 63, wave = tid >> 6;
    const int l = blockIdx.y * 16 + wave;
    for (int r0 = 0; r0 < R; r0 += RN) {
        const int rn = min(RN, R - r0), i0 = b * R + r0;
        unsigned lmask = 0;
        for (int r = 0; r < rn; ++r) if (lengths[i0 + r] > step) lmask |= 1u << r;
        __syncthreads();
        for (int e = tid; e < RN * D; e += 1024) {
            const int r = e / D, d = e - r * D; const long row = i0 + r;
            float dz = 0.f, dbp = 0.f;
            if ((lmask >> r) & 1u) {
                const float beta = hc[row * hc_ld + A + d], z = Zs[row * D + d], dx = dXZ[row * D + d];
                dz = dZ_out[row * D + d] + dx * beta;
                dbp = dx * z * beta * (1.f - beta);
            }
            s_dz[e] = dz;
            if (blockIdx.y == 0 && r < rn) { DZ[row * D + d] = dz; dhc[row * dhc_ld + A + d] = dbp; if (dhcb) dhcb[row * dhc_ld + A + d] = (__bf16)dbp; }
        }
        __syncthreads();
        if (l < L) {
            float part[RN];
#pragma unroll
            for (int r = 0; r < RN; ++r) part[r] = 0.f;
            const TA* a = ann + ((long)b * L + l) * D;
            for (int d0 = lane * 4; d0 < D; d0 += 512) {
                const int d1 = d0 + 256;
                const float4 av0 = ld_ann4<TA>(a + d0);
                const float4 av1 = d1 < D ? ld_ann4<TA>(a + d1) : make_float4(0.f, 0.f, 0.f, 0.f);
#pragma unroll
                for (int r = 0; r < RN; ++r) {
                    const float4 z0 = *reinterpret_cast<const float4*>(s_dz + r * D + d0);
                    float p = part[r];
                    p = fmaf(av0.x, z0.x, p); p = fmaf(av0.y, z0.y, p); p = fmaf(av0.z, z0.z, p); p = fmaf(av0.w, z0.w, p);
                    if (d1 < D) {
                        const float4 z1 = *reinterpret_cast<const float4*>(s_dz + r * D + d1);
                        p = fmaf(av1.x, z1.x, p); p = fmaf(av1.y, z1.y, p); p = fmaf(av1.z, z1.z, p); p = fmaf(av1.w, z1.w, p);
                    }
                    part[r] = p;
                }
            }
#pragma unroll
            for (int r = 0; r < RN; ++r) {
                const float sdot = wave_sum(part[r]);
                if (lane == 0 && r < rn)
                    da[(long)(i0 + r) * L + l] = ((lmask >> r) & 1u) ? sdot + (dalphas_ext ? dalphas_ext[((long)(i0 + r) * T1 + step) * L + l] : 0.f) : 0.f;
            }
        }
    }
}

constexpr int ATTB_KCH = 32;
template <int RN>
__global__ __launch_bounds__(1024) void attention_bwd_tanh_kernel(const float* __restrict__ U, const float* __restrict__ hc, int hc_ld, const float* __restrict__ wf,
        const int* __restrict__ lengths, int step, const float* __restrict__ alphas, int T1, const float* __restrict__ da, float* __restrict__ dhc,
        int dhc_ld, float* __restrict__ dU, float* __restrict__ dwf_part, int R, int L, int A, __bf16* __restrict__ dhcb) {
    extern __shared__ __attribute__((aligned(16))) float sm[];
    float* s_ds = sm;
    float* s_q = s_ds + RN * L;
    float* s_red = s_q + RN * ATTB_KCH;
    const int b = blockIdx.x, tid = threadIdx.x, lane = tid & 63, wave = tid >> 6;
    const int kk = tid & 31, lg = tid >> 5, k = blockIdx.y * ATTB_KCH + kk;
    const float scale = 1.0f / sqrtf((float)L);
    const float w = k < A ? wf[k] : 0.f;
    float dw_total = 0.f;
    for (int r0 = 0; r0 < R; r0 += RN) {
        const int rn = min(RN, R - r0), i0 = b * R + r0;
// ... 2 lines not shown
        __syncthreads();
        for (int r = wave; r < RN; r += 16) {
            const bool livr = (lmask >> r) & 1u;
            float dot = 0.f;
            if (livr) for (int l = lane; l < L; l += 64) dot += alphas[((long)(i0 + r) * T1 + step) * L + l] * da[(long)(i0 + r) * L + l];
            dot = wave_sum(dot);
            for (int l = lane; l < L; l += 64)
                s_ds[r * L + l] = livr ? alphas[((long)(i0 + r) * T1 + step) * L + l] * (da[(long)(i0 + r) * L + l] - dot) * scale : 0.f;
        }
        for (int e = tid; e < RN * ATTB_KCH; e += 1024) {
            const int r = e / ATTB_KCH, k2 = blockIdx.y * ATTB_KCH + (e - r * ATTB_KCH);
            s_q[e] = (((lmask >> r) & 1u) && k2 < A) ? hc[(long)(i0 + r) * hc_ld + k2] : 0.f;
        }
        __syncthreads();
        float dq[RN], dw = 0.f;
#pragma unroll
        for (int r = 0; r < RN; ++r) dq[r] = 0.f;
        if (k < A && lmask) {
            for (int l = lg; l < L; l += 32) {
                const long uo = ((long)b * L + l) * A + k;
                const float uv = U[uo];
                float du = 0.f;
#pragma unroll
                for (int r = 0; r < RN; ++r) {
                    const float th = fast_tanh(uv + s_q[r * ATTB_KCH + kk]);
                    const float ds = s_ds[r * L + l];
                    const float dp = ds * w * (1.f - th * th);
                    dq[r] += dp; du += dp; dw = fmaf(ds, th, dw);
                }
                dU[uo] += du;
            }
        }
#pragma unroll
        for (int r = 0; r < RN; ++r) s_red[(lg * (RN + 1) + r) * ATTB_KCH + kk] = dq[r];
        s_red[(lg * (RN + 1) + RN) * ATTB_KCH + kk] = dw;
        __syncthreads();
        for (int e = tid; e < (RN + 1) * ATTB_KCH; e += 1024) {
            const int r = e / ATTB_KCH, k2 = e - r * ATTB_KCH, kg = blockIdx.y * ATTB_KCH + k2;
            float sacc = 0.f;
            for (int g2 = 0; g2 < 32; ++g2) sacc += s_red[(g2 * (RN + 1) + r) * ATTB_KCH + k2];
            if (kg < A) {
                if (r < RN) { if (r < rn) { dhc[(long)(i0 + r) * dhc_ld + kg] = sacc; if (dhcb) dhcb[(long)(i0 + r) * dhc_ld + kg] = (__bf16)sacc; } }
                else s_q[k2] = sacc;
            }
        }
        __syncthreads();
        if (tid < ATTB_KCH) dw_total += s_q[tid];
    }
    if (tid < ATTB_KCH && k < A) dwf_part[(long)b * A + k] += dw_total;
}

template <int NQ>
__global__ __launch_bounds__(256) void dann_from_context_kernel(const float* __restrict__ alphas, const float* __restrict__ DZ, const int* __restrict__ lengths,
                                         float* __restrict__ dann, int accumulate, int R, int N, int T1, int L, int D) {
    extern __shared__ float4 s_a4[];
    const int b = blockIdx.x, d = blockIdx.y * blockDim.x + threadIdx.x;
    const int Lq = ((L + 3) / 4 + NQ - 1) / NQ * NQ, Lp = Lq * 4;
    float* s_a = reinterpret_cast<float*>(s_a4);
    for (int idx = threadIdx.x; idx < R * T1 * Lp; idx += blockDim.x) {
        const int row = idx / Lp, l = idx - row * Lp;
        s_a[idx] = l < L ? alphas[((long)b * R * T1 + row) * L + l] : 0.f;
    }
    __syncthreads();
    if (d >= D) return;
    for (int q0 = 0; q0 < Lq; q0 += NQ) {
        float acc[NQ * 4];
#pragma unroll
        for (int j = 0; j < NQ * 4; ++j) acc[j] = 0.f;
        for (int r = 0; r < R; ++r) {
            const int i = b * R + r; const int len = min(lengths[i], T1);
            const float4* sa = s_a4 + (long)r * T1 * Lq + q0;
            for (int t0 = 0; t0 < len; t0 += 8) {
                float dz[8];
#pragma unroll
                for (int u = 0; u < 8; ++u) dz[u] = (t0 + u < len) ? DZ[((long)(t0 + u) * N + i) * D + d] : 0.f;
#pragma unroll
                for (int u = 0; u < 8; ++u) {
                    const int tt = (t0 + u < T1) ? t0 + u : T1 - 1;
#pragma unroll
                    for (int q = 0; q < NQ; ++q) {
                        const float4 a4 = sa[tt * Lq + q];
                        acc[4 * q] = fmaf(a4.x, dz[u], acc[4 * q]); acc[4 * q + 1] = fmaf(a4.y, dz[u], acc[4 * q + 1]);
                        acc[4 * q + 2] = fmaf(a4.z, dz[u], acc[4 * q + 2]); acc[4 * q + 3] = fmaf(a4.w, dz[u], acc[4 * q + 3]);
                    }
                }
            }
        }
#pragma unroll
        for (int j = 0; j < NQ * 4; ++j) {
            const int l = q0 * 4 + j;
            if (l < L) {
                float* p = dann + ((long)b * L + l) * D + d;
                *p = accumulate ? (*p + acc[j]) : acc[j];
            }
        }
    }
}

__global__ void dann_add_mean_kernel(float* __restrict__ dann, const float* __restrict__ dmean, int L, int D, long total) {
    long e = (long)blockIdx.x * blockDim.x + threadIdx.x;
    if (e >= total) return;
    long b = e / ((long)L * D); int d = (int)(e % D);
    dann[e] += dmean[b * D + d] / (float)L;
}

__global__ void colsum_part_kernel(const float* __restrict__ x, long ld, int rows, int cols, int rows_per, float* __restrict__ part) {
    int c = blockIdx.x * blockDim.x + threadIdx.x;
    if (c >= cols) return;
    int r0 = blockIdx.y * rows_per, r1 = min(rows, r0 + rows_per);
    float s = 0.f;
    for (int r = r0; r < r1; ++r) s += x[(long)r * ld + c];
    part[(long)blockIdx.y * cols + c] = s;
}
__global__ void colsum_part4_kernel(const float* __restrict__ x, long ld, int rows, int cols4, int rows_per, float* __restrict__ part) {
    const int c4 = blockIdx.x * blockDim.x + threadIdx.x;
    if (c4 >= cols4) return;
    const int r0 = blockIdx.y * rows_per, r1 = min(rows, r0 + rows_per);
    float4 a[4];
#pragma unroll
    for (int u = 0; u < 4; ++u) a[u] = make_float4(0.f, 0.f, 0.f, 0.f);
    int r = r0;
    for (; r + 3 < r1; r += 4) {
#pragma unroll
        for (int u = 0; u < 4; ++u) {
            const float4 v = *reinterpret_cast<const float4*>(x + (long)(r + u) * ld + 4 * c4);
            a[u].x += v.x; a[u].y += v.y; a[u].z += v.z; a[u].w += v.w;
        }
    }
    for (; r < r1; ++r) { const float4 v = *reinterpret_cast<const float4*>(x + (long)r * ld + 4 * c4); a[0].x += v.x; a[0].y += v.y; a[0].z += v.z; a[0].w += v.w; }
    float4 s;
    s.x = (a[0].x + a[1].x) + (a[2].x + a[3].x); s.y = (a[0].y + a[1].y) + (a[2].y + a[3].y);
    s.z = (a[0].z + a[1].z) + (a[2].z + a[3].z); s.w = (a[0].w + a[1].w) + (a[2].w + a[3].w);
    *reinterpret_cast<float4*>(part + (long)blockIdx.y * cols4 * 4 + 4 * c4) = s;
}
// ... 131 lines not shown
```

show-attend-and-tell-pytorch-lightning_amd/csrc/decoder_step.h:

```cpp
#pragma once
#include "decoder.h"
#include "gemm.h"

namespace sat {

extern thread_local int t_bf16_mfma;

inline int gemm(hipStream_t st, int amode, int bmode, const float* A, long lda, const float* B, long ldb, float* C, long ldc,
                int M, int N, int K, int acc = 0, int epi = EPI_NONE, const float* bias = nullptr, const int* a_rows = nullptr,
                const int* c_rows = nullptr, const float* e0 = nullptr, long lde0 = 0, int c0 = 0, int c1 = 0, float* slab = nullptr, long slab_elems = 0) {
    GemmArgs g;
    g.A = A; g.lda = lda; g.B = B; g.ldb = ldb; g.C = C; g.ldc = ldc; g.M = M; g.N = N; g.K = K;
    g.amode = amode; g.bmode = bmode; g.accumulate = acc; g.epi = epi; g.bias = bias; g.a_rows = a_rows; g.c_rows = c_rows;
    g.e0 = e0; g.lde0 = lde0; g.c0 = c0; g.c1 = c1; g.slab = slab; g.slab_elems = slab_elems;
    g.bf16_mfma = t_bf16_mfma;
    return launch_gemm(g, st);
}

int pack_step_weights(const sat_decoder_dims& d, const sat_decoder_params& p, float* Wcat, __bf16* Wcat_b, float* bcat, float* bup, hipStream_t st);
int image_begin(const sat_decoder_dims& d, const sat_decoder_params& p, const float* ann, int images, float* U, float* mean, float* f, float* init_img,
                hipStream_t st);
int lstm_cell_pointwise(float* gates, int g_ld, const float* c_prev, const float* h_prev, float* c_new, float* h_new, const int* live, int rows, int n,
                        hipStream_t st);

}
```

show-attend-and-tell-pytorch-lightning_amd/csrc/gemm.h:

```cpp
#pragma once
#include "common.h"

namespace sat {

enum AMode : int {
    A_ROW = 0,
    A_KMAJOR = 1,
    A_CONV_FWD = 2,
    A_CONV_DGRAD = 3
};
enum BMode : int {
    B_ROW = 0,
    B_KMAJOR = 1,
    B_CONV_WGRAD = 2,
    B_CONV_DGRAD_W = 3
};
enum Epi : int {
    EPI_NONE = 0,
    EPI_BIAS = 1,
    EPI_BIAS_SIGMOID_RANGE = 2,
    EPI_ADD_TANH = 3,
    EPI_MUL_DTANH = 4,
    EPI_BIAS_RELU = 5
};

struct ConvGeom {
    int N, H, W, C;
    int K, R, S;
    int P, Q;
    int stride, pad;
    int sw = 0;
    int cls = 0, ph = 0, pw = 0, Hc = 0, Wc = 0, r0 = 0, rc = 0, s0 = 0, sc = 0;
};

struct GemmArgs {
    const void* A = nullptr; long lda = 0; const int* a_rows = nullptr;
    const void* B = nullptr; long ldb = 0;
    void* C = nullptr;        long ldc = 0; const int* c_rows = nullptr;
    int a_bf16 = 0, b_bf16 = 0, c_bf16 = 0;
    int bf16_mfma = 0;
    int M = 0, N = 0, K = 0;
    int amode = A_ROW, bmode = B_ROW;
    int accumulate = 0;
    int epi = EPI_NONE;
    const float* bias = nullptr;
    const float* e0 = nullptr; long lde0 = 0;
    int c0 = 0, c1 = 0;
    ConvGeom g = {};
    float* slab = nullptr; long slab_elems = 0;
    const void* bn_x = nullptr; const unsigned char* bn_mask = nullptr; const float* bn_mean = nullptr; const float* bn_invstd = nullptr;
    const void* add_src = nullptr; const unsigned char* add_mask = nullptr;
    float* tile_stats = nullptr; int* tile_rows = nullptr;
};

int launch_gemm(const GemmArgs& a, hipStream_t stream);
int launch_gemm_bf16(const GemmArgs& a, hipStream_t stream);
int gemm_bf16_eligible(const GemmArgs& a);
enum { SW_UNUSED0 = 0, SW_WGRAD3X3 = 1, SW_REDUCE_Z16 = 2, SW_WIDE_TILES = 3, SW_BN_ONEPASS = 4, SW_BN_VPT = 5, SW_ACC_PREFETCH = 6, SW_COUNT = 7 };
int& dev_switch(int which);

int wgrad3x3_eligible(const ConvGeom& g);
int launch_wgrad3x3(const void* dy, const void* x, float* dw, const ConvGeom& g, float* slab, long slab_elems, hipStream_t st);
size_t gemm_slab_bytes(int M, int N, int K);

}
```

show-attend-and-tell-pytorch-lightning_amd/csrc/gemm.hip:

```cpp
#include "gemm.h"
#include "profile.h"

namespace sat {

typedef float f32x16 __attribute__((ext_vector_type(16)));

constexpr int BK = 16;
constexpr int NTHREADS = 256;

struct KArgs {
    const float* A; long lda; const int* a_rows;
    const float* B; long ldb;
    float* C; long ldc; const int* c_rows;
    int M, N, K;
    int accumulate, epi;
    const float* bias; const float* e0; long lde0; int c0, c1;
    ConvGeom g;
    int avec, bvec;
    int kchunk, nsplit;
    float* slab;
};

__device__ __forceinline__ float epilogue_value(const KArgs& a, int row, int col, float v) {
    switch (a.epi) {
        case EPI_BIAS: v += a.bias[col]; break;
        case EPI_BIAS_SIGMOID_RANGE:
            if (a.bias) v += a.bias[col];
            if (col >= a.c0 && col < a.c1) v = fast_sigmoid(v);
            break;
        case EPI_ADD_TANH: {
            long er = a.a_rows ? (long)a.a_rows[row] : (long)row;
            v = fast_tanh(v + a.e0[er * a.lde0 + col]);
        } break;
        case EPI_MUL_DTANH: {
            float u = a.e0[(long)row * a.lde0 + col];
            v *= (1.0f - u * u);
        } break;
        case EPI_BIAS_RELU: v += a.bias[col]; v = v < 0.f ? 0.f : v; break;
        default: break;
    }
    return v;
}

__device__ __forceinline__ void store_out(const KArgs& a, int row, int col, float v) {
    long orow = row;
    if (a.c_rows) { int r = a.c_rows[row]; if (r < 0) return; orow = r; }
    float* p = a.C + orow * a.ldc + col;
    if (a.accumulate) v += *p;
    *p = epilogue_value(a, row, col, v);
}

template <int AM>
struct ARowCtx { long base; int n, y0, x0; bool ok; };

template <int AM>
__device__ __forceinline__ void a_row_setup(const KArgs& a, int m, ARowCtx<AM>& c) {
    c.ok = m < a.M; c.base = 0; c.n = c.y0 = c.x0 = 0;
    if (!c.ok) return;
    if (AM == A_ROW) {
        long r = m;
        if (a.a_rows) { int g = a.a_rows[m]; if (g < 0) { c.ok = false; return; } r = g; }
        c.base = r * a.lda;
    } else if (AM == A_CONV_FWD) {
        const ConvGeom& g = a.g;
        int pq = g.P * g.Q; c.n = m / pq; int r = m - c.n * pq; int p = r / g.Q, q = r - p * g.Q;
        c.y0 = p * g.stride - g.pad; c.x0 = q * g.stride - g.pad;
    } else {
        const ConvGeom& g = a.g;
        int hw = g.H * g.W; c.n = m / hw; int r = m - c.n * hw; int h = r / g.W, w = r - h * g.W;
        c.y0 = h + g.pad; c.x0 = w + g.pad;
    }
}

// ... 192 lines not shown
                    else store_out(a, row, col, acc[i][j][r]);
                }
            }
}

__global__ void splitk_reduce_kernel(KArgs a) {
    long idx = (long)blockIdx.x * blockDim.x + threadIdx.x;
    long total = (long)a.M * a.N;
    if (idx >= total) return;
    float v = 0.f;
    for (int z = 0; z < a.nsplit; ++z) v += a.slab[(long)z * total + idx];
    store_out(a, (int)(idx / a.N), (int)(idx % a.N), v);
}

static inline bool aligned16(const void* p) { return (reinterpret_cast<uintptr_t>(p) & 15) == 0; }

static int pick_split(int M, int N, int K, int BMt, int BNt) {
    long blocks = (long)cdiv(M, BMt) * cdiv(N, BNt);
    if (blocks >= 256 || K < 8 * BK * 2) return 1;
    int want = (int)((512 + blocks - 1) / blocks);
    int maxs = K / (8 * BK);
    int s = want < maxs ? want : maxs;
    return s < 1 ? 1 : (s > 64 ? 64 : s);
}

static void pick_tile(int M, int N, int& BMt, int& BNt) {
    long big = (long)cdiv(M, 128) * cdiv(N, 128);
    if (big >= 384 && M >= 128 && N >= 128) { BMt = BNt = 128; } else { BMt = BNt = 64; }
}

size_t gemm_slab_bytes(int M, int N, int K) {
    int BMt, BNt; pick_tile(M, N, BMt, BNt);
    int s = pick_split(M, N, K, BMt, BNt);
    return s > 1 ? (size_t)s * M * N * sizeof(float) : 0;
}

static const char* mode_name(int am, int bm) {
    if (am == A_CONV_FWD) return "conv_fwd";
    if (am == A_CONV_DGRAD) return "conv_dgrad";
    if (bm == B_CONV_WGRAD) return "conv_wgrad";
    if (am == A_ROW && bm == B_ROW) return "nt";
    if (am == A_ROW && bm == B_KMAJOR) return "nn";
    return "tn";
}

template <int BM, int BN, int AM, int BMo>
static int run(const KArgs& k, hipStream_t st) {
    dim3 grid(cdiv(k.N, BN), cdiv(k.M, BM), k.nsplit);
    char pname[96];
    if (profile_enabled()) snprintf(pname, sizeof pname, "gemm_f32_%s_%dx%d", mode_name(AM, BMo), BM, BN);
    ProfScope prof(pname, 2.0 * k.M * k.N * k.K, 4.0 * ((double)k.M * k.K + (double)k.N * k.K + (double)k.M * k.N), st);
    hipLaunchKernelGGL((gemm_f32_kernel<BM, BN, AM, BMo>), grid, dim3(NTHREADS), 0, st, k);
    SAT_TRY(launch_ok("gemm_f32_kernel"));
    if (k.nsplit > 1) {
        long total = (long)k.M * k.N;
        hipLaunchKernelGGL(splitk_reduce_kernel, dim3(cdiv(total, 256)), dim3(256), 0, st, k);
        SAT_TRY(launch_ok("splitk_reduce_kernel"));
    }
    return SAT_OK;
}

template <int AM, int BMo>
static int run_tiles(const KArgs& k, int BMt, hipStream_t st) {
    if (BMt == 128) return run<128, 128, AM, BMo>(k, st);
    return run<64, 64, AM, BMo>(k, st);
}

int launch_gemm(const GemmArgs& g, hipStream_t st) {
    SAT_REQUIRE(g.M >= 0 && g.N >= 0 && g.K >= 0, "gemm: negative dims");
    if (g.M == 0 || g.N == 0) return SAT_OK;
    SAT_REQUIRE(g.A && g.B && g.C, "gemm: null operand");
    SAT_REQUIRE(g.epi >= EPI_NONE && g.epi <= EPI_BIAS_RELU, "gemm: epi %d outside 0..%d", g.epi, (int)EPI_BIAS_RELU);
    if ((g.epi == EPI_BIAS || g.epi == EPI_BIAS_RELU) && !g.bias) return fail(SAT_EINVAL, "gemm: epilogue %d needs bias", g.epi);
    if ((g.epi == EPI_ADD_TANH || g.epi == EPI_MUL_DTANH) && !g.e0) return fail(SAT_EINVAL, "gemm: epilogue %d needs e0", g.epi);
    SAT_REQUIRE(g.slab_elems >= 0 && (g.slab || g.slab_elems == 0), "gemm: split-K slab of %ld elements at address %p", g.slab_elems, (void*)g.slab);
    if (g.bf16_mfma && gemm_bf16_eligible(g)) return launch_gemm_bf16(g, st);
    SAT_REQUIRE(!g.a_bf16 && !g.b_bf16 && !g.c_bf16, "gemm: bf16 operands need the bf16 MFMA kernel (16-byte gatherable shapes)");
    SAT_REQUIRE(!g.add_src, "gemm: add_src is a bf16-storage feature");
    KArgs k;
    k.A = (const float*)g.A; k.lda = g.lda; k.a_rows = g.a_rows; k.B = (const float*)g.B; k.ldb = g.ldb;
    k.C = (float*)g.C; k.ldc = g.ldc; k.c_rows = g.c_rows; k.M = g.M; k.N = g.N; k.K = g.K;
    k.accumulate = g.accumulate; k.epi = g.epi; k.bias = g.bias; k.e0 = g.e0; k.lde0 = g.lde0;
    k.c0 = g.c0; k.c1 = g.c1; k.g = g.g; k.slab = g.slab;
    const bool conv_a = (g.amode == A_CONV_FWD || g.amode == A_CONV_DGRAD);
    const bool conv_b = (g.bmode == B_CONV_WGRAD || g.bmode == B_CONV_DGRAD_W);
    if (conv_a || conv_b) {
        SAT_REQUIRE(g.g.C % 4 == 0 && g.g.K % 4 == 0, "conv gemm: C (%d) and K (%d) must be multiples of 4", g.g.C, g.g.K);
        SAT_REQUIRE(aligned16(g.A) && aligned16(g.B), "conv gemm: operands must be 16-byte aligned");
        SAT_REQUIRE(g.g.stride >= 1 && g.g.P > 0 && g.g.Q > 0, "conv gemm: bad geometry");
    }
    if (g.amode == A_ROW) k.avec = (g.K % 4 == 0) && (g.lda % 4 == 0) && aligned16(g.A);
    else if (g.amode == A_KMAJOR) k.avec = (g.M % 4 == 0) && (g.lda % 4 == 0) && aligned16(g.A);
    else k.avec = 1;
    if (g.bmode == B_ROW) k.bvec = (g.K % 4 == 0) && (g.ldb % 4 == 0) && aligned16(g.B);
    else if (g.bmode == B_KMAJOR) k.bvec = (g.N % 4 == 0) && (g.ldb % 4 == 0) && aligned16(g.B);
    else k.bvec = 1;

    int BMt, BNt; pick_tile(g.M, g.N, BMt, BNt);
    int ns = 1;
    if (g.slab && g.K > 0) {
        ns = pick_split(g.M, g.N, g.K, BMt, BNt);
        while (ns > 1 && (long)ns * g.M * g.N > g.slab_elems) --ns;
    }
    int ktiles = cdiv(g.K, BK);
    int per = cdiv(ktiles, ns);
    k.kchunk = per * BK;
    k.nsplit = (g.K == 0) ? 1 : cdiv(ktiles, per);
    if (k.kchunk == 0) k.kchunk = BK;

#define SAT_GEMM_CASE(AMV, BMV) \
    if (g.amode == AMV && g.bmode == BMV) return run_tiles<AMV, BMV>(k, BMt, st);
    SAT_GEMM_CASE(A_ROW, B_ROW)
    SAT_GEMM_CASE(A_ROW, B_KMAJOR)
    SAT_GEMM_CASE(A_KMAJOR, B_KMAJOR)
    SAT_GEMM_CASE(A_CONV_FWD, B_ROW)
    SAT_GEMM_CASE(A_CONV_DGRAD, B_CONV_DGRAD_W)
    SAT_GEMM_CASE(A_KMAJOR, B_CONV_WGRAD)
#undef SAT_GEMM_CASE
    return fail(SAT_EUNSUPPORTED, "gemm: operand mode pair (%d,%d) not built", g.amode, g.bmode);
}

}
```

show-attend-and-tell-pytorch-lightning_amd/csrc/gemm_bf16.hip:

```cpp
#include <stdlib.h>

#include "gemm_bf16_common.h"
#include "profile.h"

namespace sat {

struct RowCtx { long base; int n, y0, x0; bool ok; };

template <int AM>
__device__ __forceinline__ void row_setup(const BArgs& a, int m, RowCtx& c) {
    c.ok = m < a.M; c.base = 0; c.n = c.y0 = c.x0 = 0;
    if (!c.ok) return;
    if (AM == A_ROW) {
        long r = m;
        if (a.a_rows) { int g = a.a_rows[m]; if (g < 0) { c.ok = false; return; } r = g; }
        c.base = r * a.lda;
    } else if (AM == A_CONV_FWD) {
        const ConvGeom& g = a.g;
        int pq = g.P * g.Q; c.n = m / pq; int r = m - c.n * pq; int p = r / g.Q, q = r - p * g.Q;
        c.y0 = p * g.stride - g.pad; c.x0 = q * (g.sw ? g.sw : g.stride) - g.pad;
    } else {
        const ConvGeom& g = a.g;
        int h, w;
        if (g.cls) { int hw = g.Hc * g.Wc; c.n = m / hw; int r = m - c.n * hw; int hc = r / g.Wc; h = 2 * hc + g.ph; w = 2 * (r - hc * g.Wc) + g.pw; }
// ... 185 lines not shown
                    }
                }
#pragma unroll
                for (int j = 0; j < TN; ++j) {
                    if (!BKM) bf[j] = *reinterpret_cast<const bf16x8*>(bs + (wn + j * 32 + li) * LDR + kk + 8 * lh);
                    else {
                        const __bf16* p = bs + (kk + 8 * t_h + t_q) * LDB_K + wn + j * 32 + 16 * t_mh + 4 * t_p;
                        bf16x4 lo = __builtin_amdgcn_ds_read_tr16_b64_v4bf16((__attribute__((address_space(3))) bf16x4*)p);
                        bf16x4 hi = __builtin_amdgcn_ds_read_tr16_b64_v4bf16((__attribute__((address_space(3))) bf16x4*)(p + 4 * LDB_K));
                        bf[j] = __builtin_shufflevector(lo, hi, 0, 1, 2, 3, 4, 5, 6, 7);
                    }
                }
#pragma unroll
                for (int i = 0; i < TM; ++i)
#pragma unroll
                    for (int j = 0; j < TN; ++j)
                        acc[i][j] = __builtin_amdgcn_mfma_f32_32x32x16_bf16(af[i], bf[j], acc[i][j], 0, 0, 0);
            }
            if (more) stash(cur ^ 1);
            fill_tab(it & 1, k0 + 2 * KB);
            __syncthreads();
            cur ^= 1;
        }
    }

    BnAcc<BM, BN, NT> bnacc(a, bn, tid);
    store_tile<BM, BN, TC, 2 * STAGE>(a, acc, smem, bm, bn, bz, wm, wn, tid, lane, bnacc, false);
}

static const char* mname(int am, int bm) {
    if (am == A_CONV_FWD) return "conv_fwd";
    if (am == A_CONV_DGRAD) return "conv_dgrad";
    if (bm == B_CONV_WGRAD) return "conv_wgrad";
    if (am == A_ROW && bm == B_ROW) return "nt";
    if (am == A_ROW && bm == B_KMAJOR) return "nn";
    return "tn";
}

template <int AM> struct KTile { static constexpr int v = 64; };

template <int BM, int BN, int AM, int BMo, typename TA, typename TB, typename TC>
static int runb(const BArgs& k, hipStream_t st) {
    constexpr int KB = KTile<AM>::v;
    dim3 grid(cdiv(k.N, BN), cdiv(k.M, BM), k.nsplit);
    char pname[128];
    if (profile_enabled()) {
        static const bool shapes = getenv("SAT_PROFILE_SHAPES") != nullptr;
        if (shapes) snprintf(pname, sizeof pname, "gemm_bf16_%s_%dx%d_%s M%d N%d K%d z%d", mname(AM, BMo), BM, BN, sizeof(TA) == 2 ? "b" : "f", k.M, k.N, k.K, k.nsplit);
        else snprintf(pname, sizeof pname, "gemm_bf16_%s_%dx%d_%s", mname(AM, BMo), BM, BN, sizeof(TA) == 2 ? "b" : "f");
    }
    ProfScope prof(pname, 2.0 * k.M * k.N * k.K, (double)sizeof(TA) * k.M * k.K + (double)sizeof(TB) * k.N * k.K + (double)sizeof(TC) * k.M * k.N, st);
    hipLaunchKernelGGL((gemm_bf16_kernel<BM, BN, KB, AM, BMo, TA, TB, TC>), grid, dim3(NT), 0, st, k);
    SAT_TRY(launch_ok("gemm_bf16_kernel"));
    if (k.nsplit > 1) SAT_TRY(launch_splitk_reduce<TC>(k, st));
    return SAT_OK;
}

template <int AM, int BMo, typename TA, typename TB, typename TC>
static int runb_tiles(const BArgs& k, int BMt, hipStream_t st) {
    if (BMt == 128) return runb<128, 128, AM, BMo, TA, TB, TC>(k, st);
    return runb<64, 64, AM, BMo, TA, TB, TC>(k, st);
}

static inline bool al16(const void* p) { return (reinterpret_cast<uintptr_t>(p) & 15) == 0; }

int gemm_bf16_eligible(const GemmArgs& g) {
    const int va = g.a_bf16 ? 8 : 4, vb = g.b_bf16 ? 8 : 4;
    if (!al16(g.A) || !al16(g.B)) return 0;
    switch (g.amode) {
        case A_ROW: if (g.K % va || g.lda % va) return 0; break;
        case A_KMAJOR: if (g.M % va || g.lda % va) return 0; break;
        case A_CONV_FWD: if (g.g.C % va) return 0; break;
        case A_CONV_DGRAD: if (g.g.K % va) return 0; break;
        default: return 0;
    }
    switch (g.bmode) {
        case B_ROW: if (g.K % vb || g.ldb % vb) return 0; break;
        case B_KMAJOR: if (g.N % vb || g.ldb % vb) return 0; break;
        case B_CONV_WGRAD: if (g.g.C % vb) return 0; break;
        case B_CONV_DGRAD_W: if (g.g.C % vb) return 0; break;
        default: return 0;
    }
    return 1;
}

int& gemm_tile_override() { static int v = -1; return v; }

static int launch_gemm_bf16_tile(const GemmArgs& g, int tile_mode, hipStream_t st);

static int pick_wide_tile(const GemmArgs& g) {
    const int wide = dev_switch(SW_WIDE_TILES);
    if (!wide || !g.a_bf16 || !g.b_bf16 || g.a_rows || g.c_rows || g.K % 64) return 0;
    if (g.amode == A_KMAJOR && !g.c_bf16) return (g.M >= 256 && g.N >= 256 && g.K >= 4096) ? 256 : 0;
    if ((g.amode == A_CONV_FWD || (g.amode == A_ROW && g.bmode == B_ROW)) && g.c_bf16 && !g.accumulate)
        return (g.N >= 256 && g.M >= 8192 && (long)cdiv(g.M, 256) * cdiv(g.N, 128) >= 128) ? 257 : 0;
    return 0;
}

int launch_gemm_bf16(const GemmArgs& g, hipStream_t st) {
    if (g.M == 0 || g.N == 0) return SAT_OK;
    int mode = gemm_tile_override() > 0 ? gemm_tile_override() : pick_wide_tile(g);
    if (mode >= 256) {
        const int r = launch_gemm_bf16_tile(g, mode, st);
        if (r != -1) return r;
    }
    return launch_gemm_bf16_tile(g, (mode == 64 || mode == 128) ? mode : 0, st);
}

static int launch_gemm_bf16_tile(const GemmArgs& g, int tile_mode, hipStream_t st) {
    SAT_REQUIRE(g.A && g.B && g.C, "gemm_bf16: null operand");
    SAT_REQUIRE(gemm_bf16_eligible(g), "gemm_bf16: operands not 16-byte gatherable (mode %d,%d M=%d N=%d K=%d)", g.amode, g.bmode, g.M, g.N, g.K);
    BArgs k;
    k.A = g.A; k.lda = g.lda; k.a_rows = g.a_rows; k.B = g.B; k.ldb = g.ldb; k.C = g.C; k.ldc = g.ldc; k.c_rows = g.c_rows;
    k.M = g.M; k.N = g.N; k.K = g.K; k.accumulate = g.accumulate; k.epi = g.epi; k.bias = g.bias; k.e0 = g.e0; k.lde0 = g.lde0;
    k.c0 = g.c0; k.c1 = g.c1; k.g = g.g; k.slab = g.slab;
    const int KB = 64;
    int BMt = 64;
    static const long tiles128_min = getenv("SAT_TILES128_MIN") ? atol(getenv("SAT_TILES128_MIN")) : 192;
    const long tiles128 = (long)cdiv(g.M, 128) * cdiv(g.N, 128);
    if (tiles128 >= tiles128_min && g.M >= 128 && g.N >= 128) BMt = 128;
    if (BMt == 128 && tiles128 < 512 && g.K <= 256 && !g.slab) BMt = 64;
    if (g.slab && g.M >= 128 && g.N >= 128 && g.K >= 64 * KB) BMt = 128;
    if (tile_mode) BMt = tile_mode;
    const int tbm = BMt >= 256 ? 256 : BMt, tbn = BMt == 256 ? 256 : (BMt == 257 ? 128 : BMt);
    long blocks = (long)cdiv(g.M, tbm) * cdiv(g.N, tbn);
    int ns = 1;
    if (g.slab && blocks < 256 && g.K >= 16 * KB) {
        static const int target = getenv("SAT_SPLIT_TARGET") ? atoi(getenv("SAT_SPLIT_TARGET")) : 768;
        static const int frac = getenv("SAT_SPLIT_FRAC") ? atoi(getenv("SAT_SPLIT_FRAC")) : 8;
        static const int target128 = getenv("SAT_SPLIT_TARGET128") ? atoi(getenv("SAT_SPLIT_TARGET128")) : 512;
        static const int target256 = getenv("SAT_SPLIT_TARGET256") ? atoi(getenv("SAT_SPLIT_TARGET256")) : 256;
        const int tgt = (BMt >= 256) ? target256 : (BMt == 128) ? target128 : target;
        static const int floor_mode = getenv("SAT_SPLIT_FLOOR") ? atoi(getenv("SAT_SPLIT_FLOOR")) : 1;
        int want = floor_mode ? (int)(tgt / blocks) : (int)((tgt + blocks - 1) / blocks), maxs = g.K / (8 * KB);
        if (want < 1) want = 1;
        double in_bytes = ((double)g.M + g.N) * g.K * 2.0;
        int lim = (int)(in_bytes / ((double)frac * g.M * g.N)); if (lim < 4) lim = 4;
        ns = want < maxs ? want : maxs; if (ns > lim) ns = lim; if (ns > 256) ns = 256; if (ns < 1) ns = 1;
        while (ns > 1 && (long)ns * g.M * g.N > g.slab_elems) --ns;
    }
    int ktiles = cdiv(g.K, KB); if (ktiles < 1) ktiles = 1;
    int per = cdiv(ktiles, ns);
    k.kchunk = per * KB; k.nsplit = cdiv(ktiles, per);
    k.wide_store = (g.c_bf16 && !g.c_rows && k.nsplit == 1 && g.N % 8 == 0 && g.ldc % 8 == 0 && al16(g.C) &&
                    (g.epi == EPI_NONE || ((g.epi == EPI_BIAS || g.epi == EPI_BIAS_RELU) && !g.accumulate))) ? 1 : 0;
    if (!g.c_bf16 && !g.c_rows && g.N % 4 == 0 && g.ldc % 4 == 0 && al16(g.C)) k.wide_store = 1;
    k.wide_slab = (k.nsplit > 1 && g.N % 4 == 0 && al16(g.slab)) ? 1 : 0;
    k.tile_stats = nullptr;
    if (g.tile_rows) *g.tile_rows = 0;
    if (g.tile_stats && g.tile_rows && g.c_bf16 && k.wide_store && !g.accumulate && !g.g.cls && !g.bn_x) { k.tile_stats = g.tile_stats; *g.tile_rows = tbm; }
    if (g.tile_stats && g.tile_rows && g.bn_x && g.bn_mean && g.bn_invstd && g.c_bf16 && k.wide_store && k.nsplit == 1 && !g.g.cls && g.ldc == g.N &&
        g.epi == EPI_NONE && al16(g.bn_x) && BMt != 256) {
        k.tile_stats = g.tile_stats; *g.tile_rows = tbm;
        k.bn_x = reinterpret_cast<const __bf16*>(g.bn_x); k.bn_mask = g.bn_mask; k.bn_mean = g.bn_mean; k.bn_invstd = g.bn_invstd;
    }

    k.acc_prefetch = dev_switch(SW_ACC_PREFETCH);
    if (g.add_src) {
        SAT_REQUIRE(g.c_bf16 && k.wide_store && k.nsplit == 1 && g.accumulate && al16(g.add_src) && (!g.add_mask || g.ldc % 8 == 0),
                    "gemm_bf16: add_src needs an accumulating bf16 launch on the 16-byte store path (M=%d N=%d ldc=%ld)", g.M, g.N, g.ldc);
        k.add_src = reinterpret_cast<const __bf16*>(g.add_src); k.add_mask = g.add_mask;
    }
    static const bool log_shapes = getenv("SAT_LOG_GEMM") != nullptr;
    if (log_shapes) fprintf(stderr, "GEMMLOG am=%d bm=%d M=%d N=%d K=%d ns=%d acc=%d types=%d%d%d epi=%d\n", g.amode, g.bmode, g.M, g.N, g.K, k.nsplit,
                            g.accumulate, g.a_bf16, g.b_bf16, g.c_bf16, g.epi);
#define SAT_BCASE(AMV, BMV, TA, TB, TC) return runb_tiles<AMV, BMV, TA, TB, TC>(k, BMt, st);
    const bool ab = g.a_bf16, bb = g.b_bf16, cb = g.c_bf16;
    if (ab && bb) {
        int bm_used = BMt;
        const int r = launch_gemm_glds(k, g.amode, g.bmode, cb, BMt, st, &bm_used);
        if (r != -1) { if (k.tile_stats && g.tile_rows) *g.tile_rows = bm_used; return r; }
    }
    if (BMt >= 256) { if (g.tile_rows) *g.tile_rows = 0; return -1; }
    if (ab && bb) {
        if (g.amode == A_CONV_FWD && g.bmode == B_ROW && cb) SAT_BCASE(A_CONV_FWD, B_ROW, __bf16, __bf16, __bf16)
        if (g.amode == A_ROW && g.bmode == B_ROW && cb) SAT_BCASE(A_ROW, B_ROW, __bf16, __bf16, __bf16)
        if (g.amode == A_ROW && g.bmode == B_ROW && !cb) SAT_BCASE(A_ROW, B_ROW, __bf16, __bf16, float)
        if (g.amode == A_CONV_DGRAD && g.bmode == B_CONV_DGRAD_W && cb) SAT_BCASE(A_CONV_DGRAD, B_CONV_DGRAD_W, __bf16, __bf16, __bf16)
        if (g.amode == A_ROW && g.bmode == B_KMAJOR && cb) SAT_BCASE(A_ROW, B_KMAJOR, __bf16, __bf16, __bf16)
        if (g.amode == A_ROW && g.bmode == B_KMAJOR && !cb) SAT_BCASE(A_ROW, B_KMAJOR, __bf16, __bf16, float)
        if (g.amode == A_KMAJOR && g.bmode == B_CONV_WGRAD && !cb) SAT_BCASE(A_KMAJOR, B_CONV_WGRAD, __bf16, __bf16, float)
        if (g.amode == A_KMAJOR && g.bmode == B_KMAJOR && !cb) SAT_BCASE(A_KMAJOR, B_KMAJOR, __bf16, __bf16, float)
    } else if (!ab && !bb && !cb) {
        if (g.amode == A_ROW && g.bmode == B_ROW) SAT_BCASE(A_ROW, B_ROW, float, float, float)
        if (g.amode == A_ROW && g.bmode == B_KMAJOR) SAT_BCASE(A_ROW, B_KMAJOR, float, float, float)
        if (g.amode == A_KMAJOR && g.bmode == B_KMAJOR) SAT_BCASE(A_KMAJOR, B_KMAJOR, float, float, float)
    }
#undef SAT_BCASE
    return fail(SAT_EUNSUPPORTED, "gemm_bf16: combination amode=%d bmode=%d types(%d,%d,%d) not built", g.amode, g.bmode, ab, bb, cb);
}

}
```

show-attend-and-tell-pytorch-lightning_amd/csrc/gemm_bf16_common.h:

```cpp
#pragma once
#include <stdlib.h>

#include "gemm.h"

namespace sat {

typedef __bf16 bf16x8 __attribute__((ext_vector_type(8)));
typedef __bf16 bf16x4 __attribute__((ext_vector_type(4)));
typedef short s16x4 __attribute__((ext_vector_type(4)));
typedef float f32x16 __attribute__((ext_vector_type(16)));

constexpr int NT = 256;

struct BArgs {
    const void* A; long lda; const int* a_rows;
    const void* B; long ldb;
    void* C; long ldc; const int* c_rows;
    int M, N, K;
    int accumulate, epi;
    const float* bias; const float* e0; long lde0; int c0, c1;
    ConvGeom g;
    int kchunk, nsplit;
    float* slab;
    int wide_store;
    int wide_slab = 0;
    int nstage = 2;
    int rotate = 1 << 20;
    float* tile_stats = nullptr;
    const __bf16* bn_x = nullptr; const unsigned char* bn_mask = nullptr; const float* bn_mean = nullptr; const float* bn_invstd = nullptr;
    const __bf16* add_src = nullptr; const unsigned char* add_mask = nullptr;
    int acc_prefetch = 1;
    int y_fastest = 0;
};

template <typename T> struct VecN { static constexpr int n = 16 / sizeof(T); };

__device__ __forceinline__ float ep_value(const BArgs& a, int row, int col, float v) {
    switch (a.epi) {
        case EPI_BIAS: v += a.bias[col]; break;
        case EPI_BIAS_SIGMOID_RANGE:
            if (a.bias) v += a.bias[col];
            if (col >= a.c0 && col < a.c1) v = fast_sigmoid(v);
            break;
        case EPI_ADD_TANH: { long er = a.a_rows ? (long)a.a_rows[row] : (long)row; v = fast_tanh(v + a.e0[er * a.lde0 + col]); } break;
        case EPI_MUL_DTANH: { float u = a.e0[(long)row * a.lde0 + col]; v *= (1.0f - u * u); } break;
        case EPI_BIAS_RELU: v += a.bias[col]; v = v < 0.f ? 0.f : v; break;
        default: break;
    }
    return v;
}

__device__ __forceinline__ long class_row(const BArgs& a, int row) {
    const ConvGeom& g = a.g;
    int hw = g.Hc * g.Wc; int n = row / hw; int r = row - n * hw; int hc = r / g.Wc, wc = r - hc * g.Wc;
    return ((long)n * g.H + 2 * hc + g.ph) * g.W + 2 * wc + g.pw;
}

template <typename TC>
__device__ __forceinline__ void put(const BArgs& a, int row, int col, float v) {
    long orow = row;
    if (a.g.cls) orow = class_row(a, row);
    if (a.c_rows) { int r = a.c_rows[row]; if (r < 0) return; orow = r; }
    TC* p = reinterpret_cast<TC*>(a.C) + orow * a.ldc + col;
    if (a.accumulate) v += (float)*p;
    *p = (TC)ep_value(a, row, col, v);
}


template <int BM, int BN, int NTHR, bool EN = true, bool PF = true>
struct BnAcc {
    static constexpr int VPR = BN / 8, NWV = NTHR / 64, NJ0 = BM * VPR / NTHR;
    static constexpr bool BUILT = EN && NJ0 <= 8;
    static constexpr int NJ = BUILT ? NJ0 : 1;
    static_assert(NTHR % VPR == 0 && 64 % VPR == 0, "a thread keeps one column group");
    float s1[8], s2[8], mu[8];
    bf16x8 xv[PF ? NJ : 1]; unsigned mb[PF ? NJ : 1];
    bool on;
    const BArgs* ap; int bm0, bn0, tid0;
// ... 350 lines not shown
}
template <typename TC>
__global__ void splitk_reduce_b4_kernel(BArgs a) {
    const long idx4 = (long)blockIdx.x * blockDim.x + threadIdx.x;
    const long total4 = (long)a.M * a.N / 4;
    if (idx4 >= total4) return;
    float4 v = make_float4(0.f, 0.f, 0.f, 0.f);
    const float4* s4 = reinterpret_cast<const float4*>(a.slab);
#pragma unroll 4
    for (int z = 0; z < a.nsplit; ++z) { const float4 t = s4[(long)z * total4 + idx4]; v.x += t.x; v.y += t.y; v.z += t.z; v.w += t.w; }
    const long e = idx4 * 4; const int row = (int)(e / a.N), col = (int)(e % a.N);
    if (sizeof(TC) == 4 && a.wide_store && !a.g.cls) {
        float* dst = reinterpret_cast<float*>(a.C) + (long)row * a.ldc + col;
        if (a.accumulate) { const float4 old = *reinterpret_cast<const float4*>(dst); v.x += old.x; v.y += old.y; v.z += old.z; v.w += old.w; }
        if (a.epi != EPI_NONE) { v.x = ep_value(a, row, col, v.x); v.y = ep_value(a, row, col + 1, v.y); v.z = ep_value(a, row, col + 2, v.z); v.w = ep_value(a, row, col + 3, v.w); }
        *reinterpret_cast<float4*>(dst) = v;
    } else {
        put<TC>(a, row, col, v.x); put<TC>(a, row, col + 1, v.y); put<TC>(a, row, col + 2, v.z); put<TC>(a, row, col + 3, v.w);
    }
}

template <typename TC>
__global__ __launch_bounds__(256) void splitk_reduce_z16_kernel(BArgs a) {
    __shared__ float4 part[16][16];
    const int ev = threadIdx.x & 15, zl = threadIdx.x >> 4;
    const long idx4 = (long)blockIdx.x * 16 + ev;
    const long total4 = (long)a.M * a.N / 4;
    float4 v = make_float4(0.f, 0.f, 0.f, 0.f);
    if (idx4 < total4) {
        const float4* s4 = reinterpret_cast<const float4*>(a.slab);
#pragma unroll 4
        for (int z = zl; z < a.nsplit; z += 16) { const float4 t = s4[(long)z * total4 + idx4]; v.x += t.x; v.y += t.y; v.z += t.z; v.w += t.w; }
    }
    part[zl][ev] = v;
    __syncthreads();
    if (zl != 0 || idx4 >= total4) return;
#pragma unroll
    for (int l = 1; l < 16; ++l) { const float4 t = part[l][ev]; v.x += t.x; v.y += t.y; v.z += t.z; v.w += t.w; }
    const long e = idx4 * 4; const int row = (int)(e / a.N), col = (int)(e % a.N);
    if (sizeof(TC) == 4 && a.wide_store && !a.g.cls) {
        float* dst = reinterpret_cast<float*>(a.C) + (long)row * a.ldc + col;
        if (a.accumulate) { const float4 old = *reinterpret_cast<const float4*>(dst); v.x += old.x; v.y += old.y; v.z += old.z; v.w += old.w; }
        if (a.epi != EPI_NONE) { v.x = ep_value(a, row, col, v.x); v.y = ep_value(a, row, col + 1, v.y); v.z = ep_value(a, row, col + 2, v.z); v.w = ep_value(a, row, col + 3, v.w); }
        *reinterpret_cast<float4*>(dst) = v;
    } else {
        put<TC>(a, row, col, v.x); put<TC>(a, row, col + 1, v.y); put<TC>(a, row, col + 2, v.z); put<TC>(a, row, col + 3, v.w);
    }
}

template <typename TC>
inline int launch_splitk_reduce(const BArgs& k, hipStream_t st) {
    const long total = (long)k.M * k.N;
    const int z16 = dev_switch(SW_REDUCE_Z16);
    if (k.wide_slab && z16 && k.nsplit >= 32 && total / 4 / 256 < 256)
        hipLaunchKernelGGL(splitk_reduce_z16_kernel<TC>, dim3(cdiv(total / 4, 16)), dim3(256), 0, st, k);
    else if (k.wide_slab) hipLaunchKernelGGL(splitk_reduce_b4_kernel<TC>, dim3(cdiv(total / 4, 256)), dim3(256), 0, st, k);
    else hipLaunchKernelGGL(splitk_reduce_b_kernel<TC>, dim3(cdiv(total, 256)), dim3(256), 0, st, k);
    return launch_ok("splitk_reduce_b");
}

__device__ __forceinline__ void xcd_tile(int& bx, int& by, int& bz, int y_fastest = 0) {
    const unsigned total = gridDim.x * gridDim.y * gridDim.z;
    const unsigned orig = (blockIdx.z * gridDim.y + blockIdx.y) * gridDim.x + blockIdx.x;
    const unsigned q = total >> 3, r = total & 7, xcd = orig & 7, idx = orig >> 3;
    const unsigned lin = (xcd < r ? xcd * (q + 1) : r * (q + 1) + (xcd - r) * q) + idx;
    if (y_fastest) { by = lin % gridDim.y; const unsigned t2 = lin / gridDim.y; bx = t2 % gridDim.x; bz = t2 / gridDim.x; }
    else { bx = lin % gridDim.x; const unsigned t2 = lin / gridDim.x; by = t2 % gridDim.y; bz = t2 / gridDim.y; }
}

int launch_gemm_glds(const BArgs& k, int amode, int bmode, int c_bf16, int BMt, hipStream_t st, int* bm_used = nullptr);
int& glds_force_tile();
int& glds_stages8();
int& glds_tall_k();
int& glds_tall_conv();
int& glds_ablate();
int& gemm_tile_override();

}
```

show-attend-and-tell-pytorch-lightning_amd/csrc/gemm_glds_kernel.h:

```cpp
#include <stdlib.h>

#include <initializer_list>

#pragma once
#include "gemm_bf16_common.h"
#include "profile.h"

#ifndef SAT_GLDS_ABLATE
#define SAT_GLDS_ABLATE 0
#endif

namespace sat {

typedef int i32x4 __attribute__((ext_vector_type(4)));
typedef __attribute__((address_space(3))) void* lptr_t;

__device__ void raw_buffer_load_lds(i32x4 rsrc, lptr_t lds, int size, int voffset, int soffset, int offset, int aux) __asm("llvm.amdgcn.raw.buffer.load.lds");

constexpr int OOB = (int)0x80000000;

__device__ __forceinline__ i32x4 make_rsrc(const void* base) {
    const unsigned long long b = reinterpret_cast<unsigned long long>(base);
    i32x4 r;
    r[0] = (int)(unsigned)b; r[1] = (int)(unsigned)((b >> 32) & 0xFFFF);
// ... 330 lines not shown
    else store_tile_w<BM, BN, WR, WC, TC, BNS, BPF>(a, acc, smem, bm, bn, bz, wm, wn, wrow, tid, lane, bnacc, sizeof(TC) == 2);
}

static const char* gname(int am, int bm) {
    if (am == A_CONV_FWD) return "conv_fwd";
    if (am == A_CONV_DGRAD) return "conv_dgrad";
    if (bm == B_CONV_WGRAD) return "conv_wgrad";
    if (am == A_ROW && bm == B_ROW) return "nt";
    if (am == A_ROW && bm == B_KMAJOR) return "nn";
    return "tn";
}

template <int BM, int BN, int WR, int WC, int AM, int BMo, typename TC>
static int rung(const BArgs& k, hipStream_t st) {
    dim3 grid(cdiv(k.N, BN), cdiv(k.M, BM), k.nsplit);
    char pname[128];
    if (profile_enabled()) {
        static const bool shapes = getenv("SAT_PROFILE_SHAPES") != nullptr;
        if (shapes) snprintf(pname, sizeof pname, "gemm_glds_%s_%dx%d M%d N%d K%d z%d", gname(AM, BMo), BM, BN, k.M, k.N, k.K, k.nsplit);
        else snprintf(pname, sizeof pname, "gemm_glds_%s_%dx%d", gname(AM, BMo), BM, BN);
    }
    ProfScope prof(pname, 2.0 * k.M * k.N * k.K, 2.0 * k.M * k.K + 2.0 * k.N * k.K + (double)sizeof(TC) * k.M * k.N, st);
    size_t lds = (size_t)k.nstage * (BM + BN) * 64 * sizeof(__bf16);
    const size_t epi_lds = (WR == 2 && WC == 2) ? ((sizeof(TC) == 2) ? (size_t)BM * (BN + 8) * 2 + 4 * BN * 2 * 4 : (size_t)(BM / 2) * (BN + 4) * 4)
                                                : store_lds_bytes<BM, BN, WR, WC, TC>();
    if (lds < epi_lds) lds = epi_lds;
    constexpr size_t LDS_DYN_MAX = 160 * 1024 - 2560;
    SAT_REQUIRE(lds <= LDS_DYN_MAX, "gemm_glds: %zu bytes of LDS for a %dx%d tile with %d stages", lds, BM, BN, k.nstage);
    static bool attr_set = false;
    if (!attr_set) {
        SAT_CHECK_HIP(hipFuncSetAttribute(reinterpret_cast<const void*>(&gemm_glds_kernel<BM, BN, WR, WC, AM, BMo, TC>), hipFuncAttributeMaxDynamicSharedMemorySize,
                                          (int)LDS_DYN_MAX));
        attr_set = true;
    }
#ifndef SAT_GLDS_APF
#define SAT_GLDS_APF 0
#endif
    constexpr bool HAS_APF = SAT_GLDS_APF && sizeof(TC) == 2 && WR == 2 && WC == 2 && BM == 128 && BM * (BN / 8) / 256 <= 8 &&
                             ((AM == A_ROW && BMo == B_KMAJOR) || AM == A_CONV_DGRAD);
    if constexpr (HAS_APF) {
        if (k.accumulate && k.acc_prefetch && k.wide_store && k.nsplit == 1) {
            static bool attr_apf = false;
            if (!attr_apf) {
                SAT_CHECK_HIP(hipFuncSetAttribute(reinterpret_cast<const void*>(&gemm_glds_kernel<BM, BN, WR, WC, AM, BMo, TC, true>),
                                                  hipFuncAttributeMaxDynamicSharedMemorySize, (int)LDS_DYN_MAX));
                attr_apf = true;
            }
            hipLaunchKernelGGL((gemm_glds_kernel<BM, BN, WR, WC, AM, BMo, TC, true>), grid, dim3(64 * WR * WC), lds, st, k);
            return launch_ok("gemm_glds_kernel (accumulate)");
        }
    }
    hipLaunchKernelGGL((gemm_glds_kernel<BM, BN, WR, WC, AM, BMo, TC>), grid, dim3(64 * WR * WC), lds, st, k);
    SAT_TRY(launch_ok("gemm_glds_kernel"));
    if (k.nsplit > 1) SAT_TRY(launch_splitk_reduce<TC>(k, st));
    return SAT_OK;
}


#define SAT_GLDS_INSTANTIATE(FN)                                                                  \
    template int FN<A_CONV_FWD, B_ROW, __bf16>(const BArgs&, hipStream_t);                        \
    template int FN<A_ROW, B_ROW, __bf16>(const BArgs&, hipStream_t);                             \
    template int FN<A_ROW, B_ROW, float>(const BArgs&, hipStream_t);                              \
    template int FN<A_CONV_DGRAD, B_CONV_DGRAD_W, __bf16>(const BArgs&, hipStream_t);             \
    template int FN<A_ROW, B_KMAJOR, __bf16>(const BArgs&, hipStream_t);                          \
    template int FN<A_ROW, B_KMAJOR, float>(const BArgs&, hipStream_t);                           \
    template int FN<A_KMAJOR, B_CONV_WGRAD, float>(const BArgs&, hipStream_t);                    \
    template int FN<A_KMAJOR, B_KMAJOR, float>(const BArgs&, hipStream_t);

}
```

Measured before the change: 32780 captions/s.

## Fold split-K slab reductions of decoder backward GEMMs into consumer kernels

In the decoder backward time loop, the split-K GEMMs producing dXZ and dHc can now defer their reduction. The partial-sum slabs are summed directly inside the attention_bwd_dalpha and lstm_cell_bwd kernels instead of by a separate splitk_reduce launch. This removes two reduce launches per timestep and one write/read round trip of the reduced tensor. In exchange the consumer kernels read nslab partial buffers, and the slab must stay live until the consumer runs. A launch counter, a workspace-region query and a dann_lparts switch are also added.

```diff
diff --git a/include/sat_hip.h b/include/sat_hip.h
--- a/include/sat_hip.h
+++ b/include/sat_hip.h
@@ -12,6 +12,7 @@
 int sat_abi_version(void);
 int sat_debug_trace_launches(int32_t on);
 int sat_debug_option(const char* name, int32_t value);
+int sat_debug_counter(const char* name, int64_t* value);
 const char* sat_last_error(void);
 
 typedef struct sat_profile_entry {
@@ -91,6 +92,7 @@
 } sat_decoder_batch;
 
 size_t sat_decoder_workspace_bytes(const sat_decoder_dims* d);
+int sat_decoder_workspace_region(const sat_decoder_dims* d, const char* name, size_t* offset, size_t* bytes);
 
 int sat_decoder_train_fwd(const sat_decoder_dims* d, const sat_decoder_params* w, const sat_decoder_batch* b,
                           float* logits_packed, float* alphas, void* workspace, size_t workspace_bytes, void* stream);
diff --git a/show-attend-and-tell-pytorch-lightning_amd/_lib.py b/show-attend-and-tell-pytorch-lightning_amd/_lib.py
--- a/show-attend-and-tell-pytorch-lightning_amd/_lib.py
+++ b/show-attend-and-tell-pytorch-lightning_amd/_lib.py
@@ -168,9 +168,11 @@
     "sat_abi_version": (C.c_int, []),
     "sat_debug_trace_launches": (C.c_int, [C.c_int32]),
     "sat_debug_option": (C.c_int, [C.c_char_p, C.c_int32]),
+    "sat_debug_counter": (C.c_int, [C.c_char_p, C.POINTER(C.c_int64)]),
     "sat_last_error": (C.c_char_p, []),
     "sat_gemm_f32": (C.c_int, [C.POINTER(GemmDesc), C.c_void_p]),
     "sat_decoder_workspace_bytes": (C.c_size_t, [C.POINTER(DecoderDims)]),
+    "sat_decoder_workspace_region": (C.c_int, [C.POINTER(DecoderDims), C.c_char_p, C.POINTER(C.c_size_t), C.POINTER(C.c_size_t)]),
     "sat_decoder_train_fwd": (C.c_int, [C.POINTER(DecoderDims), C.POINTER(DecoderParams), C.POINTER(DecoderBatch),
                                         C.c_void_p, C.c_void_p, C.c_void_p, C.c_size_t, C.c_void_p]),
     "sat_decoder_train_bwd": (C.c_int, [C.POINTER(DecoderDims), C.POINTER(DecoderParams), C.POINTER(DecoderBatch),
diff --git a/show-attend-and-tell-pytorch-lightning_amd/csrc/api.hip b/show-attend-and-tell-pytorch-lightning_amd/csrc/api.hip
--- a/show-attend-and-tell-pytorch-lightning_amd/csrc/api.hip
+++ b/show-attend-and-tell-pytorch-lightning_amd/csrc/api.hip
@@ -14,9 +14,12 @@
                               getenv("SAT_REDUCE_Z16") ? atoi(getenv("SAT_REDUCE_Z16")) : 1, getenv("SAT_WIDE_TILES") ? atoi(getenv("SAT_WIDE_TILES")) : 0,
                               getenv("SAT_BN_ONEPASS") ? atoi(getenv("SAT_BN_ONEPASS")) : 1,
                               getenv("SAT_BN_VPT") ? atoi(getenv("SAT_BN_VPT")) : 2,
-                              getenv("SAT_ACC_PREFETCH") ? atoi(getenv("SAT_ACC_PREFETCH")) : 0};
+                              getenv("SAT_ACC_PREFETCH") ? atoi(getenv("SAT_ACC_PREFETCH")) : 0,
+                              getenv("SAT_SLAB_FOLD") ? atoi(getenv("SAT_SLAB_FOLD")) : 1,
+                              getenv("SAT_DANN_LPARTS") ? atoi(getenv("SAT_DANN_LPARTS")) : 4};
     return v[which];
 }
+std::atomic<long>& splitk_reduce_launches() { static std::atomic<long> n{0}; return n; }
 int& trace_launches() { static int on = getenv("SAT_TRACE_LAUNCH") ? 1 : 0; return on; }
 char* last_error_buf() { return g_err; }
 int fail(int code, const char* fmt, ...) {
@@ -39,12 +42,19 @@
     if (!strcmp(name, "bn_vpt")) { dev_switch(SW_BN_VPT) = value; return SAT_OK; }
     if (!strcmp(name, "bn_onepass")) { dev_switch(SW_BN_ONEPASS) = value; return SAT_OK; }
     if (!strcmp(name, "wide_tiles")) { dev_switch(SW_WIDE_TILES) = value; return SAT_OK; }
+    if (!strcmp(name, "slab_fold")) { dev_switch(SW_SLAB_FOLD) = value; return SAT_OK; }
+    if (!strcmp(name, "dann_lparts")) { dev_switch(SW_DANN_LPARTS) = value; return SAT_OK; }
     if (!strcmp(name, "glds_tile")) { glds_force_tile() = value; return SAT_OK; }
     if (!strcmp(name, "glds_stages8")) { glds_stages8() = value; return SAT_OK; }
     if (!strcmp(name, "glds_tall_k")) { glds_tall_k() = value; return SAT_OK; }
     if (!strcmp(name, "glds_tall_conv")) { glds_tall_conv() = value; return SAT_OK; }
     if (!strcmp(name, "tile_override")) { gemm_tile_override() = value; return SAT_OK; }
     return fail(SAT_EINVAL, "debug_option: unknown option %s", name);
+}
+int sat_debug_counter(const char* name, int64_t* value) {
+    if (!name || !value) return fail(SAT_EINVAL, "debug_counter: null argument");
+    if (!strcmp(name, "splitk_reduce")) { *value = (int64_t)splitk_reduce_launches().load(); return SAT_OK; }
+    return fail(SAT_EINVAL, "debug_counter: unknown counter %s", name);
 }
 const char* sat_last_error(void) { return last_error_buf(); }
 
@@ -69,6 +79,12 @@
 size_t sat_decoder_workspace_bytes(const sat_decoder_dims* d) {
     if (check_dims(d) != SAT_OK) return 0;
     return decoder_workspace_bytes(*d);
+}
+
+int sat_decoder_workspace_region(const sat_decoder_dims* d, const char* name, size_t* offset, size_t* bytes) {
+    SAT_TRY(check_dims(d));
+    if (!name || !offset || !bytes) return fail(SAT_EINVAL, "sat_decoder_workspace_region: null argument");
+    return decoder_workspace_region(*d, name, offset, bytes);
 }
 
 static int check_params(const sat_decoder_dims* d, const sat_decoder_params* w, const char* what) {
diff --git a/show-attend-and-tell-pytorch-lightning_amd/csrc/decoder.h b/show-attend-and-tell-pytorch-lightning_amd/csrc/decoder.h
--- a/show-attend-and-tell-pytorch-lightning_amd/csrc/decoder.h
+++ b/show-attend-and-tell-pytorch-lightning_amd/csrc/decoder.h
@@ -6,6 +6,7 @@
 struct Ws;
 int check_dims(const sat_decoder_dims* d);
 size_t decoder_workspace_bytes(const sat_decoder_dims& d);
+int decoder_workspace_region(const sat_decoder_dims& d, const char* name, size_t* offset, size_t* bytes);
 int decoder_fwd(const sat_decoder_dims& d, const sat_decoder_params& p, const sat_decoder_batch& b, float* logits, float* alphas,
                 char* ws, size_t ws_bytes, hipStream_t st);
 int decoder_bwd(const sat_decoder_dims& d, const sat_decoder_params& p, const sat_decoder_batch& b, const float* dlogits,
@@ -43,7 +44,8 @@
                          hipStream_t st);
 int launch_attention_bwd(hipStream_t st, const float* ann, const float* U, const float* hc, int hc_ld, const float* wf, const int* lengths, int step,
                          const float* alphas, const float* dalphas, int T1, const float* Z, const float* dZ, const float* dXZ, float* DZ, float* dhc,
-                         int dhc_ld, float* dU, float* dwf_part, float* da, int B, int R, int L, int D, int A, void* dhcb, const void* annb);
+                         int dhc_ld, float* dU, float* dwf_part, float* da, int B, int R, int L, int D, int A, void* dhcb, const void* annb,
+                         int dxz_nslab = 0, long dxz_stride = 0);
 int attention_context_bwd(const float* alphas, const float* DZ, const int* lengths, float* dann, int accumulate, int B, int R, int T1, int L, int D, hipStream_t st);
 int lstm_cell_fwd(const float* x, int in, const float* h_prev, const float* c_prev, const float* w_ih, const float* w_hh, const float* b_ih, const float* b_hh,
                   float* gates, float* h_new, float* c_new, float* bias_scratch, int N, int n, hipStream_t st);
diff --git a/show-attend-and-tell-pytorch-lightning_amd/csrc/decoder.hip b/show-attend-and-tell-pytorch-lightning_amd/csrc/decoder.hip
--- a/show-attend-and-tell-pytorch-lightning_amd/csrc/decoder.hip
+++ b/show-attend-and-tell-pytorch-lightning_amd/csrc/decoder.hip
@@ -1,5 +1,6 @@
 #include "../../include/sat_hip.h"
 #include <stdlib.h>
+#include <string.h>
 #include <map>
 #include <mutex>
 #include <utility>
@@ -124,10 +125,12 @@
     return launch_gemm(g, st);
 }
 
-static int gemm_bb_nn(hipStream_t st, const __bf16* A, long lda, const __bf16* B, long ldb, float* C, long ldc, int M, int N, int K, int acc, float* slab, long slab_elems) {
+static int gemm_bb_nn(hipStream_t st, const __bf16* A, long lda, const __bf16* B, long ldb, float* C, long ldc, int M, int N, int K, int acc, float* slab, long slab_elems,
+                      SlabInfo* defer = nullptr) {
     GemmArgs g;
     g.A = A; g.lda = lda; g.B = B; g.ldb = ldb; g.C = C; g.ldc = ldc; g.M = M; g.N = N; g.K = K;
     g.amode = A_ROW; g.bmode = B_KMAJOR; g.a_bf16 = g.b_bf16 = 1; g.c_bf16 = 0; g.bf16_mfma = 1; g.accumulate = acc; g.slab = slab; g.slab_elems = slab_elems;
+    g.defer = defer;
     return launch_gemm(g, st);
 }
 
@@ -316,7 +319,8 @@
 template <int RN, typename TA>
 static int attention_bwd_split_t(hipStream_t st, const TA* ann, const float* U, const float* hc, int hc_ld, const float* wf, const int* lengths, int step,
                                  const float* alphas, const float* dalphas, int T1, const float* Zs, const float* dZ_out, const float* dXZ, float* DZ, float* dhc,
-                                 int dhc_ld, float* dU, float* dwf_part, float* da, int B, int R, int L, int D, int A, __bf16* dhcb, const AttPlan& pl) {
+                                 int dhc_ld, float* dU, float* dwf_part, float* da, int B, int R, int L, int D, int A, __bf16* dhcb, const AttPlan& pl,
+                                 int dxz_nslab, long dxz_stride) {
     const size_t lds_a = pl.lds0, lds_t = pl.lds1;
     SAT_TRY(ensure_dynamic_lds(reinterpret_cast<const void*>(attention_bwd_dalpha_kernel<RN, TA>), lds_a));
     SAT_TRY(ensure_dynamic_lds(reinterpret_cast<const void*>(attention_bwd_tanh_kernel<RN>), lds_t));
@@ -324,7 +328,7 @@
     {
         ProfScope prof("attention_bwd_dalpha", 2.0 * N * L * D, (double)sizeof(TA) * B * L * D + 4.0 * N * (5.0 * D + 2.0 * L), st);
         hipLaunchKernelGGL((attention_bwd_dalpha_kernel<RN, TA>), dim3(B, cdiv(L, 16)), dim3(1024), lds_a, st, ann, hc, hc_ld, lengths, step, dalphas, T1, Zs, dZ_out, dXZ, DZ, dhc,
-                           dhc_ld, da, R, L, D, A, dhcb);
+                           dhc_ld, da, R, L, D, A, dhcb, dxz_nslab, dxz_stride);
         SAT_TRY(launch_ok("attention_bwd_dalpha"));
     }
     ProfScope prof("attention_bwd_tanh", 4.0 * N * L * A, 4.0 * (3.0 * B * L * A + N * (2.0 * A + 2.0 * L)), st);
@@ -332,18 +336,24 @@
                        dwf_part, R, L, A, dhcb);
     return launch_ok("attention_bwd_tanh");
 }
+static unsigned attention_bwd_flags(const float* ann, const float* da, const void* dhcb, const void* annb) {
+    return (da ? ATT_HAS_SCRATCH : 0u) | (al16(ann) && (!annb || al8(annb)) ? ATT_ANN_ALIGNED : 0u) | (dhcb || annb ? ATT_HAS_BF16 : 0u);
+}
 int launch_attention_bwd(hipStream_t st, const float* ann, const float* U, const float* hc, int hc_ld, const float* wf, const int* lengths, int step,
                          const float* alphas, const float* dalphas, int T1, const float* Zs, const float* dZ_out, const float* dXZ, float* DZ, float* dhc,
-                         int dhc_ld, float* dU, float* dwf_part, float* da, int B, int R, int L, int D, int A, void* dhcb_v, const void* annb_v) {
+                         int dhc_ld, float* dU, float* dwf_part, float* da, int B, int R, int L, int D, int A, void* dhcb_v, const void* annb_v,
+                         int dxz_nslab, long dxz_stride) {
     __bf16* dhcb = reinterpret_cast<__bf16*>(dhcb_v);
     const __bf16* annb = reinterpret_cast<const __bf16*>(annb_v);
-    const unsigned flags = (da ? ATT_HAS_SCRATCH : 0u) | (al16(ann) && (!annb || al8(annb)) ? ATT_ANN_ALIGNED : 0u) | (dhcb || annb ? ATT_HAS_BF16 : 0u);
+    const unsigned flags = attention_bwd_flags(ann, da, dhcb_v, annb_v);
     AttPlan pl;
     SAT_TRY(attention_plan(ATT_OP_BWD, R, L, D, A, hc_ld, T1, flags, pl, "attention_bwd"));
     SAT_REQUIRE(dhc_ld >= A + D, "attention_bwd: dhc_ld %d < A+D", dhc_ld);
+    SAT_REQUIRE(dxz_nslab == 0 || (pl.form == ATT_FORM_SPLIT && dxz_nslab > 0 && dxz_stride >= (long)B * R * D),
+                "attention_bwd: %d slabs of stride %ld for the %s form", dxz_nslab, dxz_stride, pl.form == ATT_FORM_SPLIT ? "split" : "single-launch");
     if (pl.form == ATT_FORM_SPLIT) {
-#define SAT_ATTB(RNV) case RNV: return annb ? attention_bwd_split_t<RNV, __bf16>(st, annb, U, hc, hc_ld, wf, lengths, step, alphas, dalphas, T1, Zs, dZ_out, dXZ, DZ, dhc, dhc_ld, dU, dwf_part, da, B, R, L, D, A, dhcb, pl) \
-                                            : attention_bwd_split_t<RNV, float>(st, ann, U, hc, hc_ld, wf, lengths, step, alphas, dalphas, T1, Zs, dZ_out, dXZ, DZ, dhc, dhc_ld, dU, dwf_part, da, B, R, L, D, A, dhcb, pl);
+#define SAT_ATTB(RNV) case RNV: return annb ? attention_bwd_split_t<RNV, __bf16>(st, annb, U, hc, hc_ld, wf, lengths, step, alphas, dalphas, T1, Zs, dZ_out, dXZ, DZ, dhc, dhc_ld, dU, dwf_part, da, B, R, L, D, A, dhcb, pl, dxz_nslab, dxz_stride) \
+                                            : attention_bwd_split_t<RNV, float>(st, ann, U, hc, hc_ld, wf, lengths, step, alphas, dalphas, T1, Zs, dZ_out, dXZ, DZ, dhc, dhc_ld, dU, dwf_part, da, B, R, L, D, A, dhcb, pl, dxz_nslab, dxz_stride);
         switch (pl.rn) { SAT_ATTB(1) SAT_ATTB(2) SAT_ATTB(3) SAT_ATTB(4) SAT_ATTB(5) SAT_ATTB(6) SAT_ATTB(7) default: SAT_ATTB(8) }
 #undef SAT_ATTB
     }
@@ -576,6 +586,13 @@
     static const int att_fused = getenv("SAT_ATT_FUSED") ? atoi(getenv("SAT_ATT_FUSED")) : 0;
     const bool use_b = w.Hb != nullptr && !att_fused;
     const __bf16* annb = (w.annb && !att_fused && ann_bf16_enabled() && al16(b.ann)) ? w.annb : nullptr;
+    bool fold = false;
+    if (ts > 0 && NL == 1 && !att_fused && dev_switch(SW_SLAB_FOLD)) {
+        AttPlan pl;
+        SAT_TRY(attention_plan(ATT_OP_BWD, d.R, d.L, D, A, HCW, T1, attention_bwd_flags(b.ann, w.DA, use_b ? w.DHCb : nullptr, annb), pl, "decoder_bwd"));
+        fold = pl.form == ATT_FORM_SPLIT;
+    }
+    SlabInfo dh_slabs, dxz_slabs;
     for (int t = ts - 1; t >= 0; --t) {
         const float* hc = w.HC + (long)t * N * HCW;
         float* dhc = w.DHC + (long)t * N * HCW;
@@ -589,17 +606,24 @@
         }
         hipLaunchKernelGGL(lstm_cell_bwd_kernel, dim3(cdiv((long)N * n, 256)), dim3(256), 0, st, hc + A + D, HCW, Cs(t, 0),
                            Cs(t + 1, 0), top == 0 ? w.dHout + (long)t * N * n : (const float*)nullptr, dHcs(0), dCcs(0), dhc + A + D, HCW, b.lengths, t, N, n,
-                           use_b ? w.DHCb + A + D : (__bf16*)nullptr);
+                           use_b ? w.DHCb + A + D : (__bf16*)nullptr, dh_slabs.nslab > 1 ? slab : (const float*)nullptr, dh_slabs.nslab > 1 ? dh_slabs.nslab : 0,
+                           dh_slabs.stride);
         SAT_TRY(launch_ok("lstm_cell_bwd"));
-        if (use_b) SAT_TRY(gemm_bb_nn(st, w.DHCb + A + D, HCW, w.Wz_b, D, w.dXZ, D, N, D, 4 * n, 0, slab, se));
-        else SAT_TRY(gemm(st, A_ROW, B_KMAJOR, dhc + A + D, HCW, p.w_ih + m, m + D, w.dXZ, D, N, D, 4 * n, 0, EPI_NONE, nullptr, nullptr, nullptr, nullptr, 0, 0, 0, slab, se));
-        SAT_TRY(launch_attention_bwd(st, b.ann, w.U, hc, HCW, p.att_f, b.lengths, t, alphas, dalphas, T1, w.Z + (long)t * N * D, w.dZout + (long)t * N * D, w.dXZ,
-                                     w.DZ + (long)t * N * D, dhc, HCW, w.dU, w.dwf_part, att_fused ? nullptr : w.DA, d.B, d.R, d.L, D, A,
-                                     use_b ? w.DHCb : nullptr, annb));
+        dh_slabs = SlabInfo();
+        SlabInfo* const dxz_defer = fold ? &dxz_slabs : nullptr;
+        dxz_slabs = SlabInfo();
+        if (use_b) SAT_TRY(gemm_bb_nn(st, w.DHCb + A + D, HCW, w.Wz_b, D, w.dXZ, D, N, D, 4 * n, 0, slab, se, dxz_defer));
+        else SAT_TRY(gemm(st, A_ROW, B_KMAJOR, dhc + A + D, HCW, p.w_ih + m, m + D, w.dXZ, D, N, D, 4 * n, 0, EPI_NONE, nullptr, nullptr, nullptr, nullptr, 0, 0, 0, slab, se,
+                          dxz_defer));
+        const bool dxz_in_slab = dxz_slabs.nslab > 1;
+        SAT_TRY(launch_attention_bwd(st, b.ann, w.U, hc, HCW, p.att_f, b.lengths, t, alphas, dalphas, T1, w.Z + (long)t * N * D, w.dZout + (long)t * N * D,
+                                     dxz_in_slab ? slab : w.dXZ, w.DZ + (long)t * N * D, dhc, HCW, w.dU, w.dwf_part, att_fused ? nullptr : w.DA, d.B, d.R, d.L, D, A,
+                                     use_b ? w.DHCb : nullptr, annb, dxz_in_slab ? dxz_slabs.nslab : 0, dxz_slabs.stride));
+        SlabInfo* const dh_defer = (fold && t > 0) ? &dh_slabs : nullptr;
         if (use_b) {
-            SAT_TRY(gemm_bb_nn(st, w.DHCb, HCW, w.Wcat_b, n, w.dHc, n, N, n, HCW, 1, slab, se));
+            SAT_TRY(gemm_bb_nn(st, w.DHCb, HCW, w.Wcat_b, n, w.dHc, n, N, n, HCW, 1, slab, se, dh_defer));
         } else if (NL == 1) {
-            SAT_TRY(gemm(st, A_ROW, B_KMAJOR, dhc, HCW, w.Wcat, n, w.dHc, n, N, n, HCW, 1, EPI_NONE, nullptr, nullptr, nullptr, nullptr, 0, 0, 0, slab, se));
+            SAT_TRY(gemm(st, A_ROW, B_KMAJOR, dhc, HCW, w.Wcat, n, w.dHc, n, N, n, HCW, 1, EPI_NONE, nullptr, nullptr, nullptr, nullptr, 0, 0, 0, slab, se, dh_defer));
         } else {
             SAT_TRY(gemm(st, A_ROW, B_KMAJOR, dhc, HCW, w.Wcat, n, dHcs(top), n, N, n, A + D, 1, EPI_NONE, nullptr, nullptr, nullptr, nullptr, 0, 0, 0, slab, se));
             SAT_TRY(gemm(st, A_ROW, B_KMAJOR, dhc + A + D, HCW, w.Wcat + (long)(A + D) * n, n, dHcs(0), n, N, n, 4 * n, 1, EPI_NONE, nullptr, nullptr, nullptr, nullptr, 0, 0, 0, slab, se));
@@ -710,6 +734,13 @@
 }
 
 size_t decoder_workspace_bytes(const sat_decoder_dims& d) { return layout(d, nullptr).total; }
+int decoder_workspace_region(const sat_decoder_dims& d, const char* name, size_t* offset, size_t* bytes) {
+    char* const base = reinterpret_cast<char*>((uintptr_t)1 << 20);
+    const Ws w = layout(d, base);
+    if (!strcmp(name, "slab")) { *offset = (size_t)((char*)w.slab - base); *bytes = (size_t)w.slab_elems * 4; return SAT_OK; }
+    if (!strcmp(name, "dXZ")) { *offset = (size_t)((char*)w.dXZ - base); *bytes = (size_t)d.B * d.R * d.D * 4; return SAT_OK; }
+    return fail(SAT_EINVAL, "decoder_workspace_region: unknown region %s", name);
+}
 
 
 static int fill_f(hipStream_t st, float* p, long n, float v) {
@@ -722,13 +753,17 @@
     AttPlan pl;
     SAT_TRY(attention_plan(ATT_OP_CONTEXT_BWD, R, L, D, 0, 0, T1, 0u, pl, "attention_context_bwd"));
     const size_t lds = pl.lds0;
-    if (pl.nq == 13) {
-        SAT_TRY(ensure_dynamic_lds(reinterpret_cast<const void*>(dann_from_context_kernel<13>), lds));
-        hipLaunchKernelGGL(dann_from_context_kernel<13>, dim3(B, cdiv(D, 256)), dim3(256), lds, st, alphas, DZ, lengths, dann, accumulate, R, B * R, T1, L, D);
-    } else {
-        SAT_TRY(ensure_dynamic_lds(reinterpret_cast<const void*>(dann_from_context_kernel<16>), lds));
-        hipLaunchKernelGGL(dann_from_context_kernel<16>, dim3(B, cdiv(D, 256)), dim3(256), lds, st, alphas, DZ, lengths, dann, accumulate, R, B * R, T1, L, D);
-    }
+    const int parts = dev_switch(SW_DANN_LPARTS);
+    const int nqp = parts >= 7 ? 2 : parts >= 4 ? 4 : parts >= 2 ? (pl.nq + 1) / 2 : pl.nq;
+    const int lq1 = (L + 3) / 4 < pl.nq ? (L + 3) / 4 : pl.nq;
+#define SAT_DANN(NQV)                                                                                                                                   \
+    case NQV:                                                                                                                                            \
+        SAT_TRY(ensure_dynamic_lds(reinterpret_cast<const void*>(dann_from_context_kernel<NQV>), lds));                                                  \
+        hipLaunchKernelGGL(dann_from_context_kernel<NQV>, dim3(B, cdiv(D, 256), cdiv(lq1, NQV)), dim3(256), lds, st, alphas, DZ, lengths, dann, accumulate, R, \
+                           B * R, T1, L, D, pl.lq);                                                                                                      \
+        break;
+    switch (nqp) { SAT_DANN(2) SAT_DANN(4) SAT_DANN(7) SAT_DANN(8) SAT_DANN(13) default: SAT_DANN(16) }
+#undef SAT_DANN
     return launch_ok("dann_from_context");
 }
 
diff --git a/show-attend-and-tell-pytorch-lightning_amd/csrc/decoder_kernels.h b/show-attend-and-tell-pytorch-lightning_amd/csrc/decoder_kernels.h
--- a/show-attend-and-tell-pytorch-lightning_amd/csrc/decoder_kernels.h
+++ b/show-attend-and-tell-pytorch-lightning_amd/csrc/decoder_kernels.h
@@ -450,14 +450,30 @@
     g[j] = gi; g[n + j] = gf; g[2 * n + j] = gg; g[3 * n + j] = go;
 }
 
+__device__ __forceinline__ float slab_sum(const float* __restrict__ p, int nslab, long stride) {
+    float t[8];
+#pragma unroll
+    for (int u = 0; u < 8; ++u) t[u] = p[(long)min(u, nslab - 1) * stride];
+    float v = 0.f;
+#pragma unroll
+    for (int u = 0; u < 8; ++u) v = u < nslab ? v + t[u] : v;
+    for (int z = 8; z < nslab; ++z) v += p[(long)z * stride];
+    return v;
+}
+
 __global__ void lstm_cell_bwd_kernel(const float* __restrict__ gates, int g_ld, const float* __restrict__ c_prev,
                                      const float* __restrict__ c_new, const float* __restrict__ dh_out,
                                      float* __restrict__ dh_carry, float* __restrict__ dc_carry,
                                      float* __restrict__ dgates, int dg_ld,
-                                     const int* __restrict__ lengths, int step, int N, int n, __bf16* __restrict__ dgb = nullptr) {
+                                     const int* __restrict__ lengths, int step, int N, int n, __bf16* __restrict__ dgb = nullptr,
+                                     const float* __restrict__ slab = nullptr, int nslab = 0, long slab_stride = 0) {
     long idx = (long)blockIdx.x * blockDim.x + threadIdx.x;
     if (idx >= (long)N * n) return;
     int i = (int)(idx / n), j = (int)(idx - (long)i * n);
+    if (nslab > 0) {
+        const float old = dh_carry[idx];
+        dh_carry[idx] = slab_sum(slab + idx, nslab, slab_stride) + old;
+    }
     float* dg = dgates + (long)i * dg_ld;
     __bf16* db = dgb ? dgb + (long)i * dg_ld : nullptr;
     if (lengths && lengths[i] <= step) {
@@ -591,7 +607,7 @@
 __global__ __launch_bounds__(1024) void attention_bwd_dalpha_kernel(const TA* __restrict__ ann, const float* __restrict__ hc, int hc_ld,
         const int* __restrict__ lengths, int step, const float* __restrict__ dalphas_ext, int T1, const float* __restrict__ Zs,
         const float* __restrict__ dZ_out, const float* __restrict__ dXZ, float* __restrict__ DZ, float* __restrict__ dhc, int dhc_ld,
-        float* __restrict__ da, int R, int L, int D, int A, __bf16* __restrict__ dhcb) {
+        float* __restrict__ da, int R, int L, int D, int A, __bf16* __restrict__ dhcb, int nslab, long slab_stride) {
     extern __shared__ __attribute__((aligned(16))) float s_dz[];
     const int b = blockIdx.x, tid = threadIdx.x, lane = tid & 63, wave = tid >> 6;
     const int l = blockIdx.y * 16 + wave;
@@ -604,8 +620,9 @@
             const int r = e / D, d = e - r * D; const long row = i0 + r;
             float dz = 0.f, dbp = 0.f;
             if ((lmask >> r) & 1u) {
-                const float beta = hc[row * hc_ld + A + d], z = Zs[row * D + d], dx = dXZ[row * D + d];
-                dz = dZ_out[row * D + d] + dx * beta;
+                const float beta = hc[row * hc_ld + A + d], z = Zs[row * D + d], dzo = dZ_out[row * D + d];
+                const float dx = nslab > 0 ? slab_sum(dXZ + row * D + d, nslab, slab_stride) : dXZ[row * D + d];
+                dz = dzo + dx * beta;
                 dbp = dx * z * beta * (1.f - beta);
             }
             s_dz[e] = dz;
@@ -714,10 +731,10 @@
 
 template <int NQ>
 __global__ __launch_bounds__(256) void dann_from_context_kernel(const float* __restrict__ alphas, const float* __restrict__ DZ, const int* __restrict__ lengths,
-                                         float* __restrict__ dann, int accumulate, int R, int N, int T1, int L, int D) {
+                                         float* __restrict__ dann, int accumulate, int R, int N, int T1, int L, int D, int Lq) {
     extern __shared__ float4 s_a4[];
     const int b = blockIdx.x, d = blockIdx.y * blockDim.x + threadIdx.x;
-    const int Lq = ((L + 3) / 4 + NQ - 1) / NQ * NQ, Lp = Lq * 4;
+    const int Lp = Lq * 4;
     float* s_a = reinterpret_cast<float*>(s_a4);
     for (int idx = threadIdx.x; idx < R * T1 * Lp; idx += blockDim.x) {
         const int row = idx / Lp, l = idx - row * Lp;
@@ -725,13 +742,13 @@
     }
     __syncthreads();
     if (d >= D) return;
-    for (int q0 = 0; q0 < Lq; q0 += NQ) {
+    for (int q0 = blockIdx.z * NQ; q0 * 4 < L; q0 += NQ * gridDim.z) {
         float acc[NQ * 4];
 #pragma unroll
         for (int j = 0; j < NQ * 4; ++j) acc[j] = 0.f;
         for (int r = 0; r < R; ++r) {
             const int i = b * R + r; const int len = min(lengths[i], T1);
-            const float4* sa = s_a4 + (long)r * T1 * Lq + q0;
+            const float4* sa = s_a4 + (long)r * T1 * Lq;
             for (int t0 = 0; t0 < len; t0 += 8) {
                 float dz[8];
 #pragma unroll
@@ -741,7 +758,7 @@
                     const int tt = (t0 + u < T1) ? t0 + u : T1 - 1;
 #pragma unroll
                     for (int q = 0; q < NQ; ++q) {
-                        const float4 a4 = sa[tt * Lq + q];
+                        const float4 a4 = sa[tt * Lq + min(q0 + q, Lq - 1)];
                         acc[4 * q] = fmaf(a4.x, dz[u], acc[4 * q]); acc[4 * q + 1] = fmaf(a4.y, dz[u], acc[4 * q + 1]);
                         acc[4 * q + 2] = fmaf(a4.z, dz[u], acc[4 * q + 2]); acc[4 * q + 3] = fmaf(a4.w, dz[u], acc[4 * q + 3]);
                     }
diff --git a/show-attend-and-tell-pytorch-lightning_amd/csrc/decoder_step.h b/show-attend-and-tell-pytorch-lightning_amd/csrc/decoder_step.h
--- a/show-attend-and-tell-pytorch-lightning_amd/csrc/decoder_step.h
+++ b/show-attend-and-tell-pytorch-lightning_amd/csrc/decoder_step.h
@@ -8,11 +8,12 @@
 
 inline int gemm(hipStream_t st, int amode, int bmode, const float* A, long lda, const float* B, long ldb, float* C, long ldc,
                 int M, int N, int K, int acc = 0, int epi = EPI_NONE, const float* bias = nullptr, const int* a_rows = nullptr,
-                const int* c_rows = nullptr, const float* e0 = nullptr, long lde0 = 0, int c0 = 0, int c1 = 0, float* slab = nullptr, long slab_elems = 0) {
+                const int* c_rows = nullptr, const float* e0 = nullptr, long lde0 = 0, int c0 = 0, int c1 = 0, float* slab = nullptr, long slab_elems = 0,
+                SlabInfo* defer = nullptr) {
     GemmArgs g;
     g.A = A; g.lda = lda; g.B = B; g.ldb = ldb; g.C = C; g.ldc = ldc; g.M = M; g.N = N; g.K = K;
     g.amode = amode; g.bmode = bmode; g.accumulate = acc; g.epi = epi; g.bias = bias; g.a_rows = a_rows; g.c_rows = c_rows;
-    g.e0 = e0; g.lde0 = lde0; g.c0 = c0; g.c1 = c1; g.slab = slab; g.slab_elems = slab_elems;
+    g.e0 = e0; g.lde0 = lde0; g.c0 = c0; g.c1 = c1; g.slab = slab; g.slab_elems = slab_elems; g.defer = defer;
     g.bf16_mfma = t_bf16_mfma;
     return launch_gemm(g, st);
 }
diff --git a/show-attend-and-tell-pytorch-lightning_amd/csrc/gemm.h b/show-attend-and-tell-pytorch-lightning_amd/csrc/gemm.h
--- a/show-attend-and-tell-pytorch-lightning_amd/csrc/gemm.h
+++ b/show-attend-and-tell-pytorch-lightning_amd/csrc/gemm.h
@@ -1,4 +1,6 @@
 #pragma once
+#include <atomic>
+
 #include "common.h"
 
 namespace sat {
@@ -33,6 +35,8 @@
     int cls = 0, ph = 0, pw = 0, Hc = 0, Wc = 0, r0 = 0, rc = 0, s0 = 0, sc = 0;
 };
 
+struct SlabInfo { int nslab = 1; long stride = 0; };
+
 struct GemmArgs {
     const void* A = nullptr; long lda = 0; const int* a_rows = nullptr;
     const void* B = nullptr; long ldb = 0;
@@ -48,6 +52,7 @@
     int c0 = 0, c1 = 0;
     ConvGeom g = {};
     float* slab = nullptr; long slab_elems = 0;
+    SlabInfo* defer = nullptr;
     const void* bn_x = nullptr; const unsigned char* bn_mask = nullptr; const float* bn_mean = nullptr; const float* bn_invstd = nullptr;
     const void* add_src = nullptr; const unsigned char* add_mask = nullptr;
     float* tile_stats = nullptr; int* tile_rows = nullptr;
@@ -56,8 +61,9 @@
 int launch_gemm(const GemmArgs& a, hipStream_t stream);
 int launch_gemm_bf16(const GemmArgs& a, hipStream_t stream);
 int gemm_bf16_eligible(const GemmArgs& a);
-enum { SW_UNUSED0 = 0, SW_WGRAD3X3 = 1, SW_REDUCE_Z16 = 2, SW_WIDE_TILES = 3, SW_BN_ONEPASS = 4, SW_BN_VPT = 5, SW_ACC_PREFETCH = 6, SW_COUNT = 7 };
+enum { SW_UNUSED0 = 0, SW_WGRAD3X3 = 1, SW_REDUCE_Z16 = 2, SW_WIDE_TILES = 3, SW_BN_ONEPASS = 4, SW_BN_VPT = 5, SW_ACC_PREFETCH = 6, SW_SLAB_FOLD = 7, SW_DANN_LPARTS = 8, SW_COUNT = 9 };
 int& dev_switch(int which);
+std::atomic<long>& splitk_reduce_launches();
 
 int wgrad3x3_eligible(const ConvGeom& g);
 int launch_wgrad3x3(const void* dy, const void* x, float* dw, const ConvGeom& g, float* slab, long slab_elems, hipStream_t st);
diff --git a/show-attend-and-tell-pytorch-lightning_amd/csrc/gemm.hip b/show-attend-and-tell-pytorch-lightning_amd/csrc/gemm.hip
--- a/show-attend-and-tell-pytorch-lightning_amd/csrc/gemm.hip
+++ b/show-attend-and-tell-pytorch-lightning_amd/csrc/gemm.hip
@@ -19,6 +19,7 @@
     int avec, bvec;
     int kchunk, nsplit;
     float* slab;
+    int defer_reduce;
 };
 
 __device__ __forceinline__ float epilogue_value(const KArgs& a, int row, int col, float v) {
@@ -317,8 +318,9 @@
     ProfScope prof(pname, 2.0 * k.M * k.N * k.K, 4.0 * ((double)k.M * k.K + (double)k.N * k.K + (double)k.M * k.N), st);
     hipLaunchKernelGGL((gemm_f32_kernel<BM, BN, AM, BMo>), grid, dim3(NTHREADS), 0, st, k);
     SAT_TRY(launch_ok("gemm_f32_kernel"));
-    if (k.nsplit > 1) {
+    if (k.nsplit > 1 && !k.defer_reduce) {
         long total = (long)k.M * k.N;
+        ++splitk_reduce_launches();
         hipLaunchKernelGGL(splitk_reduce_kernel, dim3(cdiv(total, 256)), dim3(256), 0, st, k);
         SAT_TRY(launch_ok("splitk_reduce_kernel"));
     }
@@ -339,6 +341,7 @@
     if ((g.epi == EPI_BIAS || g.epi == EPI_BIAS_RELU) && !g.bias) return fail(SAT_EINVAL, "gemm: epilogue %d needs bias", g.epi);
     if ((g.epi == EPI_ADD_TANH || g.epi == EPI_MUL_DTANH) && !g.e0) return fail(SAT_EINVAL, "gemm: epilogue %d needs e0", g.epi);
     SAT_REQUIRE(g.slab_elems >= 0 && (g.slab || g.slab_elems == 0), "gemm: split-K slab of %ld elements at address %p", g.slab_elems, (void*)g.slab);
+    if (g.defer) *g.defer = SlabInfo();
     if (g.bf16_mfma && gemm_bf16_eligible(g)) return launch_gemm_bf16(g, st);
     SAT_REQUIRE(!g.a_bf16 && !g.b_bf16 && !g.c_bf16, "gemm: bf16 operands need the bf16 MFMA kernel (16-byte gatherable shapes)");
     SAT_REQUIRE(!g.add_src, "gemm: add_src is a bf16-storage feature");
@@ -372,6 +375,8 @@
     k.kchunk = per * BK;
     k.nsplit = (g.K == 0) ? 1 : cdiv(ktiles, per);
     if (k.kchunk == 0) k.kchunk = BK;
+    k.defer_reduce = (g.defer && k.nsplit > 1 && g.epi == EPI_NONE && !g.c_rows) ? 1 : 0;
+    if (k.defer_reduce) { g.defer->nslab = k.nsplit; g.defer->stride = (long)g.M * g.N; }
 
 #define SAT_GEMM_CASE(AMV, BMV) \
     if (g.amode == AMV && g.bmode == BMV) return run_tiles<AMV, BMV>(k, BMt, st);
diff --git a/show-attend-and-tell-pytorch-lightning_amd/csrc/gemm_bf16.hip b/show-attend-and-tell-pytorch-lightning_amd/csrc/gemm_bf16.hip
--- a/show-attend-and-tell-pytorch-lightning_amd/csrc/gemm_bf16.hip
+++ b/show-attend-and-tell-pytorch-lightning_amd/csrc/gemm_bf16.hip
@@ -261,7 +261,7 @@
     ProfScope prof(pname, 2.0 * k.M * k.N * k.K, (double)sizeof(TA) * k.M * k.K + (double)sizeof(TB) * k.N * k.K + (double)sizeof(TC) * k.M * k.N, st);
     hipLaunchKernelGGL((gemm_bf16_kernel<BM, BN, KB, AM, BMo, TA, TB, TC>), grid, dim3(NT), 0, st, k);
     SAT_TRY(launch_ok("gemm_bf16_kernel"));
-    if (k.nsplit > 1) SAT_TRY(launch_splitk_reduce<TC>(k, st));
+    if (k.nsplit > 1 && !k.defer_reduce) SAT_TRY(launch_splitk_reduce<TC>(k, st));
     return SAT_OK;
 }
 
@@ -355,6 +355,8 @@
                     (g.epi == EPI_NONE || ((g.epi == EPI_BIAS || g.epi == EPI_BIAS_RELU) && !g.accumulate))) ? 1 : 0;
     if (!g.c_bf16 && !g.c_rows && g.N % 4 == 0 && g.ldc % 4 == 0 && al16(g.C)) k.wide_store = 1;
     k.wide_slab = (k.nsplit > 1 && g.N % 4 == 0 && al16(g.slab)) ? 1 : 0;
+    k.defer_reduce = (g.defer && k.nsplit > 1 && !g.c_bf16 && g.epi == EPI_NONE && !g.c_rows && !g.g.cls && k.wide_slab) ? 1 : 0;
+    if (g.defer) { *g.defer = SlabInfo(); if (k.defer_reduce) { g.defer->nslab = k.nsplit; g.defer->stride = (long)g.M * g.N; } }
     k.tile_stats = nullptr;
     if (g.tile_rows) *g.tile_rows = 0;
     if (g.tile_stats && g.tile_rows && g.c_bf16 && k.wide_store && !g.accumulate && !g.g.cls && !g.bn_x) { k.tile_stats = g.tile_stats; *g.tile_rows = tbm; }
diff --git a/show-attend-and-tell-pytorch-lightning_amd/csrc/gemm_bf16_common.h b/show-attend-and-tell-pytorch-lightning_amd/csrc/gemm_bf16_common.h
--- a/show-attend-and-tell-pytorch-lightning_amd/csrc/gemm_bf16_common.h
+++ b/show-attend-and-tell-pytorch-lightning_amd/csrc/gemm_bf16_common.h
@@ -24,6 +24,7 @@
     float* slab;
     int wide_store;
     int wide_slab = 0;
+    int defer_reduce = 0;
     int nstage = 2;
     int rotate = 1 << 20;
     float* tile_stats = nullptr;
@@ -480,6 +481,7 @@
 inline int launch_splitk_reduce(const BArgs& k, hipStream_t st) {
     const long total = (long)k.M * k.N;
     const int z16 = dev_switch(SW_REDUCE_Z16);
+    ++splitk_reduce_launches();
     if (k.wide_slab && z16 && k.nsplit >= 32 && total / 4 / 256 < 256)
         hipLaunchKernelGGL(splitk_reduce_z16_kernel<TC>, dim3(cdiv(total / 4, 16)), dim3(256), 0, st, k);
     else if (k.wide_slab) hipLaunchKernelGGL(splitk_reduce_b4_kernel<TC>, dim3(cdiv(total / 4, 256)), dim3(256), 0, st, k);
diff --git a/show-attend-and-tell-pytorch-lightning_amd/csrc/gemm_glds_kernel.h b/show-attend-and-tell-pytorch-lightning_amd/csrc/gemm_glds_kernel.h
--- a/show-attend-and-tell-pytorch-lightning_amd/csrc/gemm_glds_kernel.h
+++ b/show-attend-and-tell-pytorch-lightning_amd/csrc/gemm_glds_kernel.h
@@ -406,7 +406,7 @@
     }
     hipLaunchKernelGGL((gemm_glds_kernel<BM, BN, WR, WC, AM, BMo, TC>), grid, dim3(64 * WR * WC), lds, st, k);
     SAT_TRY(launch_ok("gemm_glds_kernel"));
-    if (k.nsplit > 1) SAT_TRY(launch_splitk_reduce<TC>(k, st));
+    if (k.nsplit > 1 && !k.defer_reduce) SAT_TRY(launch_splitk_reduce<TC>(k, st));
     return SAT_OK;
 }
 
```

Result: no change. 32920 captions/s (median of 6 runs) (+0.4%).
